# helloybz/CLANE

Measured on AMD Instinct MI355X. Metric: embedding-update iters/sec (Jacobi sweeps of Z <- X + gamma*P*Z, P frozen), higher is better.
Workload: dtype f32; 1 GPU; R-MAT |V|=2000000 |E|=40000000 d=256 f32, gamma=0.76, CosineSimilarity (reference mode), seeds 3/4

## Files before the change

clane_amd/_hip.py:

```python
from __future__ import annotations

import abc
import ctypes as C
import os
import threading
from pathlib import Path
from typing import Optional

import torch

LIB_NAME = "libclane_hip.so"
LIB_PATH = Path(__file__).resolve().parent / LIB_NAME
ABI_VERSION = 5

SCORE_REFERENCE, SCORE_PER_EDGE, SCORE_RAW_DOT = 0, 1, 2
SPMM_SINKS_UNTOUCHED = 1
SPMM_TABLE_BEYOND_CACHE = 2
SCORE_FUSE_SOFTMAX = 1
SCORE_MODES = {"reference": SCORE_REFERENCE, "per_edge": SCORE_PER_EDGE, "raw_dot": SCORE_RAW_DOT}

_p, _i64, _i32 = C.c_void_p, C.c_int64, C.c_int32

SIGNATURES = {
    "clane_abi_version": (C.c_int, []),
    "clane_last_error": (C.c_char_p, []),
    "clane_build_info": (C.c_char_p, []),
    "clane_xcc_ids": (C.c_int, [_p, _i64, _i32, _p]),
    "clane_check_csr": (C.c_int, [_p, _p, _i64, _i64, _i64, _p, _p]),
    "clane_spmm_partials_len": (_i64, [_i64, _i64]),
    "clane_reduce_ws_len": (_i64, []),
    "clane_reduce_partials": (C.c_int, [_p, _i64, _p, _p, _p]),
    "clane_spmm_split_slab_len": (_i64, [_i64, _i32]),
    "clane_spmm_class_slab_len": (_i64, [_i64, _i32]),
    "clane_device_alloc": (C.c_int, [_i64, C.POINTER(_p)]),
    "clane_device_alloc_contiguous": (C.c_int, [_i64, C.POINTER(_p)]),
    "clane_device_free": (C.c_int, [_p]),
    "clane_ipc_export": (C.c_int, [_p, _p]),
    "clane_ipc_open": (C.c_int, [_p, C.POINTER(_p)]),
    "clane_ipc_close": (C.c_int, [_p]),
}
IPC_HANDLE_BYTES = 64
for _s in ("f32", "f64", "bf16"):
    SIGNATURES[f"clane_row_sqnorm_{_s}"] = (C.c_int, [_p, _i64, _i32, _i64, _p, _p])
    SIGNATURES[f"clane_edge_score_{_s}"] = (
        C.c_int, [_p, _p, _i64, _i64, _p, _i64, _i32, _i32, _p, _p, _p, _i32, _i64, _p, _i64, _p])
    _g = C.c_double if _s == "f64" else C.c_float
    SIGNATURES[f"clane_spmm_update_{_s}"] = (
        C.c_int, [_p, _p, _p, _i64, _i64, _p, _i64, _p, _i64, _g, _p, _i64, _i32, _i64, _i32, _p, _p, _p])
    SIGNATURES[f"clane_spmm_update_long_{_s}"] = (
        C.c_int, [_p, _p, _p, _p, _i64, _i32, _i64, _p, _i64, _p, _i64, _g, _p, _i64, _i32, _p, _p, _p])
    SIGNATURES[f"clane_spmm_update_split_{_s}"] = (
        C.c_int,
        [_p, _p, _p, _p, _p, _p, _i64, _i64, _i64, _i64, _p, _i64, _p, _i64, _g, _p, _i64, _i32, _p, _p, _p, _p])
    SIGNATURES[f"clane_spmm_update_class_{_s}"] = (
        C.c_int,
        [_p, _p, _p, _p, _p, _i64, _i32, _p, _p, _i64, _i64, _p, _i64, _p, _i64, _g, _p, _i64, _i32, _i32, _p, _p, _p, _p])
    SIGNATURES[f"clane_edge_score_class_{_s}"] = (
        C.c_int, [_p, _p, _p, _p, _p, _p, _i64, _i32, _p, _p, _i64, _i64, _p, _i64, _i32, _i32, _p, _p, _p, _i32, _p, _p])
    SIGNATURES[f"clane_gather_rows_{_s}"] = (C.c_int, [_p, _i64, _p, _i64, _i32, _p, _i64, _p])
    SIGNATURES[f"clane_l1_distance_{_s}"] = (C.c_int, [_p, _i64, _p, _i64, _i64, _i32, _p, _p, _p, _p])
for _s in ("f32", "f64"):
    SIGNATURES[f"clane_degree_weighted_sums_{_s}"] = (C.c_int, [_p, _p, _p, _i64, _p, _p, _p])
    SIGNATURES[f"clane_edge_score_finalize_{_s}"] = (C.c_int, [_p, _p, _i64, _i64, _i32, _p, _p, _p, _p])
    SIGNATURES[f"clane_segment_softmax_{_s}"] = (C.c_int, [_p, _i64, _p, _i64, _i64, _p, _i64, _p])
    SIGNATURES[f"clane_pair_cosine_{_s}"] = (C.c_int, [_p, _i64, _p, _i64, _i64, _i32, _p, _p, _p])
    SIGNATURES[f"clane_edge_score_pair_{_s}"] = (
        C.c_int, [_p, _p, _i64, _i64, _p, _i64, _p, _i64, _i32, _p, _i32, _i64, _p, _i64, _p])
    SIGNATURES[f"clane_edge_score_class_pair_{_s}"] = (
        C.c_int, [_p, _p, _p, _p, _p, _p, _i64, _i32, _p, _p, _i64, _i64, _p, _i64, _p, _i64, _i32, _p, _i32, _p, _p])
for _s in ("f32", "f64", "bf16"):
    SIGNATURES[f"clane_project_rows_{_s}"] = (C.c_int, [_p, _i64, _i32, _i64, _p, _p, _i64, _p])
    SIGNATURES[f"clane_pair_project_{_s}"] = (C.c_int, [_p, _i64, _i32, _i64, _p, _p, _i64, _p, _p, _p, _p])
    SIGNATURES[f"clane_pair_grad_{_s}"] = (C.c_int, [_p, _i64, _i32, _i64, _p, _p, _i64, _p, _p, _p, _p, _p, _p, _p])
for _s in ("f32", "f64"):
    SIGNATURES[f"clane_pair_loss_{_s}"] = (C.c_int, [_p, _p, _i64, _i32, _p, _p, _p, _p, _p, _p, _p])
    SIGNATURES[f"clane_adam_step_{_s}"] = (C.c_int, [_p, _p, _p, _p, _i64, C.c_double, _p, _p, _p])
SIGNATURES["clane_pair_grad_ws_len"] = (_i64, [_i64, _i32])
RANK_MAX_K = 32
for _s in ("f32", "f64", "bf16"):
    SIGNATURES[f"clane_rank_scores_{_s}"] = (
        C.c_int, [_p, _i64, _p, _i64, _i64, _i32, _p, _i64, _i32, _p, _p, _p, _p, _p, _i32, _i32, _i32, _p, _p, _p])
    SIGNATURES[f"clane_pair_score_{_s}"] = (C.c_int, [_p, _i64, _p, _i64, _i64, _i32, _p, _p, _i64, _i32, _p, _p, _p, _p])
    SIGNATURES[f"clane_rank_count_{_s}"] = (
        C.c_int, [_p, _i64, _p, _i64, _i64, _i32, _p, _p, _i64, _i32, _p, _p, _p, _p, _p, _i32, _i32, _p, _p, _p])
for _s in ("f32", "f64"):
    SIGNATURES[f"clane_rank_merge_{_s}"] = (C.c_int, [_p, _p, _i64, _i32, _i32, _p, _p, _p])
SIGNATURES["clane_pair_labels"] = (C.c_int, [_p, _p, _i64, _p, _p, _i64, _p, _p])
PROBE_MAX_CLASSES = 64
PROBE_WRITE_G, PROBE_WRITE_PRED = 1, 2
PROBE_PRED_TOPK = 4
for _s in ("f32", "f64", "bf16"):
    SIGNATURES[f"clane_probe_forward_{_s}"] = (
        C.c_int, [_p, _i64, _i32, _i64, _p, _p, _i64, _p, _i64, _p, _p, _i32, _i32, _i32, _p, _p, _p, _p, _i64, _p])
    SIGNATURES[f"clane_probe_grad_{_s}"] = (C.c_int, [_p, _i64, _i32, _i64, _p, _i64, _p, _i32, _p, _p, _p, _p])
    SIGNATURES[f"clane_probe_forward_ovr_{_s}"] = (
        C.c_int, [_p, _i64, _i32, _i64, _p, _p, _i64, _p, _i64, _p, _p, _p, _i32, _i32, _i32, _i32, _p, _p, _p, _p, _i64, _p])
SIGNATURES["clane_probe_loss_ws_len"] = (_i64, [_i64, _i32])
SIGNATURES["clane_probe_grad_ws_len"] = (_i64, [_i64, _i32, _i32])
for _s in ("f32", "f64", "bf16"):
    SIGNATURES[f"clane_kmeans_assign_{_s}"] = (
        C.c_int, [_p, _i64, _i32, _i64, _p, _i64, _p, _p, _i32, _i32, _p, _i64, _p, _i64, _p])
    SIGNATURES[f"clane_kmeans_update_{_s}"] = (
        C.c_int, [_p, _i64, _i32, _i64, _p, _p, _i64, _i32, _i32, _p, _p, _p, _p, _p])
SIGNATURES["clane_kmeans_update_ws_len"] = (_i64, [_i64, _i32, _i32, _i32])
for _s in ("f32", "f64", "bf16"):
    _g = C.c_double if _s == "f64" else C.c_float
    SIGNATURES[f"clane_embed_rows_{_s}"] = (
        C.c_int, [_p, _p, _i64, _p, _i64, _p, _i64, _i64, _i32, _i32, _p, _p, _p, _i64, _g, _i32, _i32, _i32, _p, _i64,
                  _p, _p, _p, _p])

PCA_ACCUMULATE = 1
for _s in ("f32", "f64", "bf16"):
    SIGNATURES[f"clane_column_sums_{_s}"] = (C.c_int, [_p, _i64, _i32, _i64, _p, _i64, _i32, _p, _p, _p])
    SIGNATURES[f"clane_gram_{_s}"] = (C.c_int, [_p, _i64, _i32, _i64, _p, _i64, _p, _i32, _p, _p, _p])
    SIGNATURES[f"clane_project_affine_{_s}"] = (C.c_int, [_p, _i64, _i32, _i64, _p, _i64, _p, _p, _i32, _p, _i64, _p])
SIGNATURES["clane_column_sums_ws_len"] = (_i64, [_i64, _i32])
SIGNATURES["clane_gram_ws_len"] = (_i64, [_i64, _i32])


def probe_padded_classes(C_: int) -> int:
    if not 2 <= int(C_) <= PROBE_MAX_CLASSES:
        raise ValueError(f"the label probe handles 2..{PROBE_MAX_CLASSES} classes, got {C_}")
    return 1 << (int(C_) - 1).bit_length()


def ovr_padded_classes(C_: int) -> int:
    if not 1 <= int(C_) <= PROBE_MAX_CLASSES:
        raise ValueError(f"the multi-label probe handles 1..{PROBE_MAX_CLASSES} classes, got {C_}")
    return 1 << (int(C_) - 1).bit_length()


_SUFFIX = {torch.float32: "f32", torch.float64: "f64", torch.bfloat16: "bf16"}
_ACC = {torch.float32: torch.float32, torch.float64: torch.float64, torch.bfloat16: torch.float32}
VEC_ELEMS = {torch.float32: 4, torch.float64: 2, torch.bfloat16: 8}


class ClaneHipError(RuntimeError):
    pass


class _MirrorStruct(C.Structure):
    _fields_ = [("row_ptr", _p), ("slot", _p), ("bufs", _p), ("ld", _i64), ("aligned16", _i32)]

# ... 14 lines not shown
        if len({ld for _, ld in mats}) != 1 or len({b.dtype for b in bufs}) != 1:
            raise ValueError("Mirror: the buffers must share dtype and leading dimension")
        if max(b.shape[0] for b in bufs) > (1 << MIRROR_ROW_BITS):
            raise ValueError("Mirror: a buffer has more than 2^28 rows")
        self.row_ptr, self.slot, self.bufs = row_ptr, slot, bufs
        self.buf = bufs[0]
        self.bases = torch.tensor([ptr for ptr, _ in mats], dtype=torch.int64, device=row_ptr.device)
        self.c = _MirrorStruct(row_ptr.data_ptr(), slot.data_ptr(), self.bases.data_ptr(), mats[0][1],
                               int(all(ptr % 16 == 0 for ptr, _ in mats)))


class _RawDeviceMemory:

    def __init__(self, ptr: int, nbytes: int):
        self.__cuda_array_interface__ = {"shape": (nbytes,), "typestr": "|u1", "data": (ptr, False), "version": 2}


class PeerMatrix:

    def __init__(self, ptr: int, shape, dtype: torch.dtype):
        self._ptr, self.shape, self.dtype = ptr, tuple(shape), dtype

    def data_ptr(self) -> int:
        return self._ptr

    def dim(self) -> int:
        return len(self.shape)

    def stride(self, i: Optional[int] = None):
        st = (self.shape[1], 1)
        return st if i is None else st[i]


class DeviceBuffer:

    def __init__(self, lib, shape, dtype: torch.dtype, device, _mapped_from: Optional[bytes] = None,
                 contiguous: bool = False):
        self.lib, self.shape, self.dtype = lib, tuple(int(x) for x in shape), dtype
        self.nbytes = max(16, int(torch.empty(0, dtype=dtype).element_size()) * int(torch.Size(self.shape).numel()))
        self.mapped = _mapped_from is not None
        ptr = _p()
        with torch.cuda.device(device):
            if self.mapped:
                rc = lib.clane_ipc_open(_mapped_from, C.byref(ptr))
            elif contiguous:
                rc = lib.clane_device_alloc_contiguous(self.nbytes, C.byref(ptr))
            else:
                rc = lib.clane_device_alloc(self.nbytes, C.byref(ptr))
        if rc != 0:
            raise ClaneHipError(f"{'clane_ipc_open' if self.mapped else 'clane_device_alloc'} failed ({rc}): "
                                f"{lib.clane_last_error().decode()}")
        self.ptr = ptr.value
        if self.mapped:
            self.tensor = PeerMatrix(self.ptr, self.shape, dtype)
        else:
            raw = torch.as_tensor(_RawDeviceMemory(self.ptr, self.nbytes), device=torch.device(device))
            n = int(torch.Size(self.shape).numel()) * torch.empty(0, dtype=dtype).element_size()
            self.tensor = raw[:n].view(dtype).view(self.shape)
            self.tensor.zero_()

    def export(self) -> bytes:
        handle = C.create_string_buffer(IPC_HANDLE_BYTES)
        rc = self.lib.clane_ipc_export(self.ptr, handle)
        if rc != 0:
            raise ClaneHipError(f"clane_ipc_export failed ({rc}): {self.lib.clane_last_error().decode()}")
        return handle.raw

    @classmethod
    def open(cls, lib, handle: bytes, shape, dtype: torch.dtype, device) -> "DeviceBuffer":
        return cls(lib, shape, dtype, device, _mapped_from=handle)

    def close(self) -> None:
        if self.ptr:
            (self.lib.clane_ipc_close if self.mapped else self.lib.clane_device_free)(self.ptr)
            self.ptr = 0

    def __del__(self):
        try:
            self.close()
        except Exception:
            pass


def _mirror_arg(mirror: Optional["Mirror"], dtype: torch.dtype):
    if mirror is None:
        return None
    if mirror.buf.dtype != dtype:
        raise ValueError("mirror.buf must have the dtype of Z_new")
    return C.cast(C.pointer(mirror.c), _p)


def load_library(path: Optional[Path] = None) -> C.CDLL:
    if path is None and os.environ.get("CLANE_HIP_LIB"):
        path = os.environ["CLANE_HIP_LIB"]
    path = Path(path) if path is not None else LIB_PATH
    if not path.exists():
        raise ClaneHipError(
            f"{path} not found: the HIP extension is not built. Run `python -c 'import __graft_entry__ as g; "
            f"g.build()'` (or `make -C clane_amd/csrc`) -- clane_amd has no CPU fallback.")
    lib = C.CDLL(str(path))
    for name, (res, args) in SIGNATURES.items():
        fn = getattr(lib, name)
        fn.restype, fn.argtypes = res, args
    got = lib.clane_abi_version()
    if got != ABI_VERSION:
        raise ClaneHipError(f"{path}: ABI version {got}, expected {ABI_VERSION}")
    return lib


def acc_dtype(dtype: torch.dtype) -> torch.dtype:
    try:
        return _ACC[dtype]
    except KeyError:
        raise TypeError(f"clane_amd supports float32, float64 and bfloat16 embeddings, not {dtype}") from None


def _ptr(t: Optional[torch.Tensor]):
    return None if t is None else t.data_ptr()


def _mat(t: torch.Tensor, name: str):
    if t.dim() != 2 or t.stride(1) != 1:
        raise ValueError(f"{name}: need a row-major 2-D tensor with unit column stride, got {tuple(t.shape)} "
                         f"strides {t.stride()}")
    return t.data_ptr(), t.stride(0)


def _vec(t: torch.Tensor, dtype: torch.dtype, name: str):
    if t.dtype != dtype or not t.is_contiguous():
        raise ValueError(f"{name}: need a contiguous {dtype} tensor, got {t.dtype} contiguous={t.is_contiguous()}")
    return t.data_ptr()


class KernelBackend(abc.ABC):

    @abc.abstractmethod
    def spmm_partials_len(self, nrows: int, n_long: int) -> int: ...
    @abc.abstractmethod
    def reduce_ws_len(self) -> int: ...
    @abc.abstractmethod
    def spmm_split_slab_len(self, n_segments: int, d: int) -> int: ...
    @abc.abstractmethod
    def spmm_class_slab_len(self, n_slots: int, d: int) -> int: ...
    @abc.abstractmethod
    def check_csr(self, rowptr, colidx, nrows: int, n_edges: int, table_rows: int) -> None: ...
    @abc.abstractmethod
    def build_info(self) -> str: ...
    @abc.abstractmethod
    def row_sqnorm(self, Z, d: int, sq): ...
    @abc.abstractmethod
    def degree_weighted_sums(self, sq, rowptr, indeg, nrows: int, ws, out2): ...
    @abc.abstractmethod
    def edge_score(self, rowptr, colidx, nrows, row0, Z, d, mode, sums2, sq, scores, long_threshold=0, long_rows=None,
                   fuse_softmax=False): ...
    @abc.abstractmethod
    def edge_score_class(self, rowptr, colidx, item_e0, item_len, item_slot, item_row, items_per_block, class_rows,
                         slot_ptr, row0, Z, d, mode, sums2, sq, scores, stats=None, fuse_softmax=False,
                         n_slots=None, row_parts=1): ...
    @abc.abstractmethod
    def edge_score_finalize(self, rowptr, colidx, nrows, row0, mode, sums2, sq, scores): ...
    @abc.abstractmethod
    def segment_softmax(self, rowptr, nrows, vals, min_degree=0, max_degree=0, long_rows=None): ...
    @abc.abstractmethod
    def pair_cosine(self, A, B, d, out, ws): ...
    @abc.abstractmethod
    def spmm_update(self, rowptr, colidx, P, nrows, row0, Z_old, X, gamma, Z_new, d, long_threshold, partials,
# ... 25 lines not shown
    def project_rows(self, Z, d: int, W, Y):
        raise NotImplementedError(f"{type(self).__name__} has no project_rows")

    def edge_score_pair(self, rowptr, colidx, nrows, row0, S, N, d, scores, long_threshold=0, long_rows=None,
                        fuse_softmax=False):
        raise NotImplementedError(f"{type(self).__name__} has no edge_score_pair")

    def edge_score_class_pair(self, rowptr, colidx, item_e0, item_len, item_slot, item_row, items_per_block,
                              class_rows, slot_ptr, row0, S, N, d, scores, stats=None, fuse_softmax=False,
                              n_slots=None, row_parts=1):
        raise NotImplementedError(f"{type(self).__name__} has no edge_score_class_pair")

    def pair_project(self, Z, d: int, src, dst, W, A, Bm):
        raise NotImplementedError(f"{type(self).__name__} has no pair_project")

    def pair_loss(self, A, Bm, d: int, linked, u, g, mask, ws, stats):
        raise NotImplementedError(f"{type(self).__name__} has no pair_loss")

    def pair_grad_ws_len(self, B: int, d: int) -> int:
        raise NotImplementedError(f"{type(self).__name__} has no pair_grad_ws_len")

    def pair_grad(self, Z, d: int, src, dst, A, Bm, g, stats, ws, dW):
        raise NotImplementedError(f"{type(self).__name__} has no pair_grad")

    def adam_step(self, W, m, v, dW, lr: float, stats, state):
        raise NotImplementedError(f"{type(self).__name__} has no adam_step")

    def pair_labels(self, rowptr, colidx, nrows: int, src, dst, linked):
        raise NotImplementedError(f"{type(self).__name__} has no pair_labels")

    def rank_scores(self, S, N, table_rows: int, d: int, q_rows, mode: int, sums2, sq, label, excl_rowptr, excl_colidx,
                    exclude_self: bool, k: int, n_slabs: int, cand_score, cand_id):
        raise NotImplementedError(f"{type(self).__name__} has no rank_scores")

    def rank_merge(self, cand_score, cand_id, n_slabs: int, k: int, out_score, out_id):
        raise NotImplementedError(f"{type(self).__name__} has no rank_merge")

    def pair_score(self, S, N, table_rows: int, d: int, src, dst, mode: int, sums2, sq, out):
        raise NotImplementedError(f"{type(self).__name__} has no pair_score")

    def rank_count(self, S, N, table_rows: int, d: int, q_rows, t_rows, mode: int, sums2, sq, label, excl_rowptr,
                   excl_colidx, exclude_self: bool, n_slabs: int, target_score, counts):
        raise NotImplementedError(f"{type(self).__name__} has no rank_count")

    def probe_loss_ws_len(self, n: int, F: int) -> int:
        raise NotImplementedError(f"{type(self).__name__} has no probe_loss_ws_len")

    def probe_forward(self, Z, d: int, rows, y, split, W, bias, F: int, C: int, loss_ws, loss, G=None, pred=None):
        raise NotImplementedError(f"{type(self).__name__} has no probe_forward")

    def probe_forward_ovr(self, Z, d: int, rows, ymask, split, W, bias, col_state, F: int, C: int, max_labels: int,
                          loss_ws, loss, G=None, pred=None, top_k: bool = True):
        raise NotImplementedError(f"{type(self).__name__} has no probe_forward_ovr")

    def probe_grad_ws_len(self, n: int, K: int, d: int) -> int:
        raise NotImplementedError(f"{type(self).__name__} has no probe_grad_ws_len")

    def probe_grad(self, Z, d: int, rows, G, ws, dW, db):
        raise NotImplementedError(f"{type(self).__name__} has no probe_grad")

    def kmeans_assign(self, Z, d: int, rows, centres, csq, assign, best):
        raise NotImplementedError(f"{type(self).__name__} has no kmeans_assign")

    def kmeans_update_ws_len(self, n: int, R: int, K: int, d: int) -> int:
        raise NotImplementedError(f"{type(self).__name__} has no kmeans_update_ws_len")

    def kmeans_update(self, Z, d: int, order, seg, centres_old, ws, centres_new, csq_new):
        raise NotImplementedError(f"{type(self).__name__} has no kmeans_update")

    def column_sums_ws_len(self, n: int, d: int) -> int:
        raise NotImplementedError(f"{type(self).__name__} has no column_sums_ws_len")

    def column_sums(self, Z, d: int, rows, ws, sums, accumulate: bool = False):
        raise NotImplementedError(f"{type(self).__name__} has no column_sums")

    def gram_ws_len(self, n: int, d: int) -> int:
        raise NotImplementedError(f"{type(self).__name__} has no gram_ws_len")

    def gram(self, Z, d: int, rows, mu, ws, G, accumulate: bool = False):
        raise NotImplementedError(f"{type(self).__name__} has no gram")

    def project_affine(self, Z, d: int, rows, mu, W, Y):
        raise NotImplementedError(f"{type(self).__name__} has no project_affine")

    def bind(self, method: str, *args, **kwargs):
        fn = getattr(self, method)
        return lambda: fn(*args, **kwargs)

    def embed_rows(self, rowptr, colidx, X_new, Z, table_rows: int, d: int, mode: int, sums2, sq, S, gamma: float,
                   tolerence: int, max_rounds: int, Z_out, rounds, delta, P_out=None, flags: int = 0):
        raise NotImplementedError(f"{type(self).__name__} has no embed_rows")


class HipKernels(KernelBackend):

    def __init__(self, lib: Optional[C.CDLL] = None):
        self.lib = lib if lib is not None else load_library()
        self._tls = threading.local()

    def _invoke(self, fn, what: str, *cargs):
        rec = getattr(self._tls, "recording", None)
        if rec is not None:
            rec.append((fn, cargs, what))
        else:
            self._check(fn(*cargs), what)

    def bind(self, method: str, *args, **kwargs):
        self._tls.recording = []
        try:
            getattr(self, method)(*args, **kwargs)
            (fn, cargs, what), = self._tls.recording
        finally:
            self._tls.recording = None
        check = self._check
        return lambda: check(fn(*cargs), what)

    def _check(self, rc: int, what: str):
        if rc != 0:
            raise ClaneHipError(f"{what} failed ({rc}): {self.lib.clane_last_error().decode()}")

    @staticmethod
    def _stream(t: torch.Tensor):
        if not t.is_cuda:
            raise ClaneHipError("HipKernels needs tensors in GPU memory (got a CPU tensor); there is no CPU path")
        return torch.cuda.current_stream(t.device).cuda_stream

    def _fn(self, base: str, dtype: torch.dtype):
        try:
            return getattr(self.lib, f"{base}_{_SUFFIX[dtype]}")
        except KeyError:
            raise TypeError(f"{base}: unsupported dtype {dtype}") from None

    def spmm_partials_len(self, nrows: int, n_long: int) -> int:
        return int(self.lib.clane_spmm_partials_len(nrows, n_long))

    def xcc_ids(self, n_blocks: int, block_threads: int = 256, device=None) -> torch.Tensor:
        out = torch.full((n_blocks,), -1, dtype=torch.int32, device=device if device is not None else "cuda")
        self._check(self.lib.clane_xcc_ids(out.data_ptr(), n_blocks, block_threads, self._stream(out)), "clane_xcc_ids")
        return out

    def check_csr(self, rowptr: torch.Tensor, colidx: torch.Tensor, nrows: int, n_edges: int, table_rows: int) -> None:
        if rowptr.dtype != torch.int64 or colidx.dtype != torch.int32 or rowptr.numel() < nrows + 1 or colidx.numel() < n_edges:
            raise ValueError("check_csr: rowptr must be int64 [nrows + 1], colidx int32 [n_edges]")
        status = torch.zeros(1, dtype=torch.int32, device=rowptr.device)
        self._check(self.lib.clane_check_csr(rowptr.data_ptr(), colidx.data_ptr(), nrows, n_edges, table_rows,
                                             status.data_ptr(), self._stream(rowptr)), "clane_check_csr")
        bad = int(status.item())
        if bad:
            what = [w for bit, w in ((1, "rowptr is not a non-decreasing sequence within [0, n_edges]"),
                                     (2, f"colidx holds entries outside [0, {table_rows})")) if bad & bit]
            raise ValueError("the CSR handed to the kernels is not valid: " + "; ".join(what))

    def build_info(self) -> str:
        return self.lib.clane_build_info().decode()

    def make_mirror(self, row_ptr, slot, bufs) -> Mirror:
        return Mirror(row_ptr, slot, bufs)

    def reduce_ws_len(self) -> int:
        return int(self.lib.clane_reduce_ws_len())

    def contiguous_matrix(self, shape, dtype: torch.dtype, device) -> DeviceBuffer:
        return DeviceBuffer(self.lib, shape, dtype, device, contiguous=True)

    def shareable_matrix(self, shape, dtype: torch.dtype, device) -> DeviceBuffer:
        return DeviceBuffer(self.lib, shape, dtype, device)
# ... 42 lines not shown
            _vec(scores, acc, "scores"),
            (SCORE_FUSE_SOFTMAX | ((max(1, min(255, int(row_parts))) & 0xff) << 8)) if fuse_softmax else 0,
            None if stats is None else _vec(stats, acc, "stats"), self._stream(Z)), "clane_edge_score_class")

    def edge_score_finalize(self, rowptr, colidx, nrows: int, row0: int, mode: int, sums2, sq, scores):
        self._check(self._fn("clane_edge_score_finalize", scores.dtype)(
            _vec(rowptr, torch.int64, "rowptr"), _vec(colidx, torch.int32, "colidx"), nrows, row0, mode,
            _ptr(sums2), _ptr(sq), scores.data_ptr(), self._stream(scores)), "clane_edge_score_finalize")

    def segment_softmax(self, rowptr, nrows: int, vals, min_degree: int = 0, max_degree: int = 0, long_rows=None):
        n_long = 0 if long_rows is None else long_rows.numel()
        self._check(self._fn("clane_segment_softmax", vals.dtype)(
            _vec(rowptr, torch.int64, "rowptr"), nrows, vals.data_ptr(), min_degree, max_degree,
            None if n_long == 0 else _vec(long_rows, torch.int32, "long_rows"), n_long, self._stream(vals)),
            "clane_segment_softmax")

    @staticmethod
    def _sq_arg(sq: Optional[torch.Tensor], dtype: torch.dtype):
        return None if sq is None else _vec(sq, acc_dtype(dtype), "sq_a")

    def spmm_update(self, rowptr, colidx, P, nrows: int, row0: int, Z_old, X, gamma: float, Z_new, d: int,
                    long_threshold: int, partials, sinks_untouched: bool = False, mirror: Optional[Mirror] = None,
                    beyond_cache: bool = False):
        zo, ldz = _mat(Z_old, "Z_old")
        xp, ldx = _mat(X, "X")
        zn, ldo = _mat(Z_new, "Z_new")
        if not (Z_old.dtype == X.dtype == Z_new.dtype):
            raise ValueError("spmm_update: Z_old, X, Z_new must share a dtype")
        self._invoke(self._fn("clane_spmm_update", Z_old.dtype), "clane_spmm_update",
                     _vec(rowptr, torch.int64, "rowptr"), _vec(colidx, torch.int32, "colidx"),
                     _vec(P, acc_dtype(Z_old.dtype), "P"), nrows, row0, zo, ldz, xp, ldx, gamma, zn, ldo, d,
                     long_threshold, (SPMM_SINKS_UNTOUCHED if sinks_untouched else 0) | (SPMM_TABLE_BEYOND_CACHE if beyond_cache else 0),
                     _mirror_arg(mirror, Z_new.dtype), _vec(partials, torch.float64, "partials"), self._stream(Z_old))

    def spmm_update_long(self, rowptr, colidx, P, long_rows, waves_per_row: int, row0: int, Z_old, X, gamma: float,
                         Z_new, d: int, partials, mirror: Optional[Mirror] = None):
        zo, ldz = _mat(Z_old, "Z_old")
        xp, ldx = _mat(X, "X")
        zn, ldo = _mat(Z_new, "Z_new")
        if not (Z_old.dtype == X.dtype == Z_new.dtype):
            raise ValueError("spmm_update_long: Z_old, X, Z_new must share a dtype")
        self._invoke(self._fn("clane_spmm_update_long", Z_old.dtype), "clane_spmm_update_long",
                     _vec(rowptr, torch.int64, "rowptr"), _vec(colidx, torch.int32, "colidx"),
                     _vec(P, acc_dtype(Z_old.dtype), "P"), _vec(long_rows, torch.int32, "long_rows"),
                     long_rows.numel(), waves_per_row, row0, zo, ldz, xp, ldx, gamma, zn, ldo, d,
                     _mirror_arg(mirror, Z_new.dtype), _vec(partials, torch.float64, "partials"), self._stream(Z_old))

    def spmm_split_slab_len(self, n_segments: int, d: int) -> int:
        return int(self.lib.clane_spmm_split_slab_len(n_segments, d))

    def spmm_update_split(self, rowptr, colidx, P, split_rows, seg_ptr, seg_row, edges_per_segment: int, row0: int,
                          Z_old, X, gamma: float, Z_new, d: int, slab, partials, mirror: Optional[Mirror] = None):
        zo, ldz = _mat(Z_old, "Z_old")
        xp, ldx = _mat(X, "X")
        zn, ldo = _mat(Z_new, "Z_new")
        self._invoke(self._fn("clane_spmm_update_split", Z_old.dtype), "clane_spmm_update_split",
                     _vec(rowptr, torch.int64, "rowptr"), _vec(colidx, torch.int32, "colidx"),
                     _vec(P, acc_dtype(Z_old.dtype), "P"), _vec(split_rows, torch.int32, "split_rows"),
                     _vec(seg_ptr, torch.int64, "seg_ptr"), _vec(seg_row, torch.int32, "seg_row"),
                     split_rows.numel(), seg_row.numel(), edges_per_segment, row0, zo, ldz, xp, ldx, gamma, zn, ldo, d,
                     _vec(slab, acc_dtype(Z_old.dtype), "slab"), _mirror_arg(mirror, Z_new.dtype),
                     _vec(partials, torch.float64, "partials"), self._stream(Z_old))

    def spmm_class_slab_len(self, n_slots: int, d: int) -> int:
        return int(self.lib.clane_spmm_class_slab_len(n_slots, d))

    def spmm_update_class(self, colidx, P, item_e0, item_len, item_slot, items_per_block: int, class_rows, slot_ptr,
                          row0: int, Z_old, X, gamma: float, Z_new, d: int, slab, partials,
                          mirror: Optional[Mirror] = None, beyond_cache: bool = False):
        zo, ldz = _mat(Z_old, "Z_old")
        xp, ldx = _mat(X, "X")
        zn, ldo = _mat(Z_new, "Z_new")
        n_items = item_e0.numel()
        if n_items % items_per_block or item_len.numel() != n_items or item_slot.numel() != n_items:
            raise ValueError("spmm_update_class: the item arrays must hold whole blocks of items_per_block items")
        self._invoke(self._fn("clane_spmm_update_class", Z_old.dtype), "clane_spmm_update_class",
                     _vec(colidx, torch.int32, "colidx"), _vec(P, acc_dtype(Z_old.dtype), "P"),
                     _vec(item_e0, torch.int64, "item_e0"), _vec(item_len, torch.int32, "item_len"),
                     _vec(item_slot, torch.int32, "item_slot"), n_items // items_per_block, items_per_block,
                     _vec(class_rows, torch.int32, "class_rows"), _vec(slot_ptr, torch.int64, "slot_ptr"),
                     class_rows.numel(), row0, zo, ldz, xp, ldx, gamma, zn, ldo, d,
                     SPMM_TABLE_BEYOND_CACHE if beyond_cache else 0,
                     _vec(slab, acc_dtype(Z_old.dtype), "slab"), _mirror_arg(mirror, Z_new.dtype),
                     _vec(partials, torch.float64, "partials"), self._stream(Z_old))

    def reduce_partials(self, partials, n: int, ws, out):
        self._invoke(self.lib.clane_reduce_partials, "clane_reduce_partials",
                     _vec(partials, torch.float64, "partials"), n, _vec(ws, torch.float64, "ws"),
                     _vec(out, torch.float64, "out"), self._stream(out))

    def l1_distance(self, A, B, d: int, ws, out, sq_a: Optional[torch.Tensor] = None):
        ap, lda = _mat(A, "A")
        bp, ldb = _mat(B, "B")
        self._check(self._fn("clane_l1_distance", A.dtype)(
            ap, lda, bp, ldb, A.shape[0], d, self._sq_arg(sq_a, A.dtype), _vec(ws, torch.float64, "ws"),
            _vec(out, torch.float64, "out"), self._stream(A)), "clane_l1_distance")

    def gather_rows(self, src, idx, d: int, dst):
        sp, lds = _mat(src, "src")
        dp, ldd = _mat(dst, "dst")
        self._invoke(self._fn("clane_gather_rows", src.dtype), "clane_gather_rows",
                     sp, lds, _vec(idx, torch.int32, "idx"), idx.numel(), d, dp, ldd, self._stream(src))

    def project_rows(self, Z, d: int, W, Y):
        zp, ldz = _mat(Z, "Z")
        yp, ldy = _mat(Y, "Y")
        acc = acc_dtype(Z.dtype)
        if tuple(W.shape) != (2 * d, d):
            raise ValueError(f"project_rows: W must be [2d, d] = [{2 * d}, {d}], got {tuple(W.shape)}")
        if Y.dtype != acc or Y.shape[0] < Z.shape[0]:
            raise ValueError(f"project_rows: Y must be {acc} with at least {Z.shape[0]} rows")
        self._check(self._fn("clane_project_rows", Z.dtype)(
            zp, Z.shape[0], d, ldz, _vec(W, acc, "W"), yp, ldy, self._stream(Z)), "clane_project_rows")

    def edge_score_pair(self, rowptr, colidx, nrows: int, row0: int, S, N, d: int, scores, long_threshold: int = 0,
                        long_rows=None, fuse_softmax: bool = False):
        sp, lds = _mat(S, "S")
        np_, ldn = _mat(N, "N")
        if S.dtype != N.dtype:
            raise ValueError("edge_score_pair: S and N must share a dtype")
        n_long = 0 if long_rows is None else long_rows.numel()
        self._check(self._fn("clane_edge_score_pair", S.dtype)(
            _vec(rowptr, torch.int64, "rowptr"), _vec(colidx, torch.int32, "colidx"), nrows, row0, sp, lds, np_, ldn, d,
            _vec(scores, S.dtype, "scores"), SCORE_FUSE_SOFTMAX if fuse_softmax else 0, long_threshold,
            None if n_long == 0 else _vec(long_rows, torch.int32, "long_rows"), n_long,
            self._stream(S)), "clane_edge_score_pair")

    def edge_score_class_pair(self, rowptr, colidx, item_e0, item_len, item_slot, item_row, items_per_block: int,
                              class_rows, slot_ptr, row0: int, S, N, d: int, scores, stats=None,
                              fuse_softmax: bool = False, n_slots: Optional[int] = None, row_parts: int = 1):
        sp, lds = _mat(S, "S")
        np_, ldn = _mat(N, "N")
        if S.dtype != N.dtype:
            raise ValueError("edge_score_class_pair: S and N must share a dtype")
        n_items = item_e0.numel()
        if n_items % items_per_block or any(t.numel() != n_items for t in (item_len, item_slot, item_row)):
            raise ValueError("edge_score_class_pair: the item arrays must hold whole blocks of items_per_block items")
        if fuse_softmax and (stats is None or stats.numel() < 2 * (int(slot_ptr[-1]) if n_slots is None else n_slots)):
            raise ValueError("edge_score_class_pair: stats needs 2 elements per slot")
        self._check(self._fn("clane_edge_score_class_pair", S.dtype)(
            _vec(rowptr, torch.int64, "rowptr"), _vec(colidx, torch.int32, "colidx"),
            _vec(item_e0, torch.int64, "item_e0"), _vec(item_len, torch.int32, "item_len"),
            _vec(item_slot, torch.int32, "item_slot"), _vec(item_row, torch.int32, "item_row"),
            n_items // items_per_block, items_per_block, _vec(class_rows, torch.int32, "class_rows"),
            _vec(slot_ptr, torch.int64, "slot_ptr"), class_rows.numel(), row0, sp, lds, np_, ldn, d,
            _vec(scores, S.dtype, "scores"),
            (SCORE_FUSE_SOFTMAX | ((max(1, min(255, int(row_parts))) & 0xff) << 8)) if fuse_softmax else 0,
            None if stats is None else _vec(stats, S.dtype, "stats"), self._stream(S)), "clane_edge_score_class_pair")

    @staticmethod
    def _pairs(src, dst, what: str) -> int:
        if src.numel() != dst.numel():
            raise ValueError(f"{what}: src and dst must have one entry per pair")
        return src.numel()

    def _pair_mats(self, A, Bm, B: int, d: int, acc, what: str):
        for t, name in ((A, "A"), (Bm, "Bm")):
            if t.dtype != acc or not t.is_contiguous() or t.numel() < B * d:
                raise ValueError(f"{what}: {name} must be a contiguous {acc} tensor of at least B * d elements")
        return A.data_ptr(), Bm.data_ptr()

    def pair_project(self, Z, d: int, src, dst, W, A, Bm):
        zp, ldz = _mat(Z, "Z")
        acc = acc_dtype(Z.dtype)
        B = self._pairs(src, dst, "pair_project")
        if tuple(W.shape) != (2 * d, d):
# ... 322 lines not shown
```

clane_amd/csrc/clane_abi.hip:

```cpp
#include "../../include/clane_hip.h"

#include <hip/hip_runtime.h>

#include <climits>
#include <cstdarg>
#include <cstdio>
#include <cstring>

#include "build_p.h"
#include "content_pca.h"
#include "edge_score.h"
#include "device_utils.h"
#include "kmeans.h"
#include "label_probe.h"
#include "multilabel_probe.h"
#include "new_rows.h"
#include "link_eval.h"
#include "link_rank.h"
#include "pair_train.h"
#include "projection.h"
#include "spmm_update.h"

namespace {

// ... 393 lines not shown
        else
            spmm_long_kernel<T, PT, VEC, LPR, U, kLongWaves>
                <<<int(n_long), kLongWaves * kWave, 0, (hipStream_t)stream>>>(
                    rowptr, colidx, P, long_rows, row0, Z_old, ldz, X, ldx, gamma, Z_new, ldo, d, mir, delta_partials);
    });
    return check_launch("spmm_update_long");
}

template <typename T, typename PT>
int spmm_update_split(const int64_t *rowptr, const int32_t *colidx, const PT *P, const int32_t *split_rows,
                      const int64_t *seg_ptr, const int32_t *seg_row, int64_t n_split, int64_t n_segments,
                      int64_t edges_per_segment, int64_t row0, const T *Z_old, int64_t ldz, const T *X, int64_t ldx,
                      typename Elem<T>::acc_t gamma, T *Z_new, int64_t ldo, int32_t d,
                      typename Elem<T>::acc_t *slab, const clane_mirror_t *mirror, double *delta_partials,
                      void *stream) {
    REQUIRE(mirror_ok(mirror, d), "spmm_update_split: incomplete mirror descriptor");
    REQUIRE(n_split >= 0 && n_split <= INT32_MAX && n_segments >= n_split && n_segments <= INT32_MAX && row0 >= 0 &&
                d > 0 && edges_per_segment >= kWave && edges_per_segment % kWave == 0,
            "spmm_update_split: bad shape (edges_per_segment must be a positive multiple of 64)");
    REQUIRE(ldz >= d && ldx >= d && ldo >= d, "spmm_update_split: leading dimension < d");
    if (n_split == 0) return CLANE_OK;
    REQUIRE(rowptr && colidx && P && split_rows && seg_ptr && seg_row && Z_old && X && Z_new && slab && delta_partials,
            "spmm_update_split: null pointer");
    REQUIRE((const void *)Z_new != (const void *)Z_old, "spmm_update_split: Z_new must not alias Z_old");
    REQUIRE(aligned16(slab), "spmm_update_split: slab must be 16-byte aligned");
    const Layout L = pick_layout<T>(d, {Z_old, X, Z_new, mirror_alignment_probe(mirror, Z_new)},
                                    {ldz, ldx, ldo, mirror && mirror->row_ptr ? mirror->ld : ldo});
    const int64_t ld_slab = ceil_div(d, 8) * 8;
    const Mirror<T> mir = make_mirror<T>(mirror);
    dispatch_layout<T>(L, [&]<int VEC, int LPR>() {
        constexpr int U = VEC > 1 ? CLANE_LONG_U : 4;
        spmm_split_segment_kernel<T, PT, VEC, LPR, U, kLongWaves>
            <<<unsigned(n_segments), kLongWaves * kWave, 0, (hipStream_t)stream>>>(
                rowptr, colidx, P, split_rows, seg_ptr, seg_row, edges_per_segment, Z_old, ldz, d, slab, ld_slab);
        spmm_class_combine_kernel<T, VEC, LPR>
            <<<unsigned(ceil_div(n_split, kWave / LPR)), kCombineWaves * kWave, 0, (hipStream_t)stream>>>(
            split_rows, seg_ptr, n_split, row0, slab, ld_slab, Z_old, ldz, X, ldx, gamma, Z_new, ldo, d, mir, false, delta_partials);
    });
    return check_launch("spmm_update_split");
}

template <typename T, typename PT>
int spmm_update_class(const int32_t *colidx, const PT *P, const int64_t *item_e0, const int32_t *item_len,
                      const int32_t *item_slot, int64_t n_blocks, int32_t items_per_block, const int32_t *class_rows,
                      const int64_t *slot_ptr, int64_t n_rows, int64_t row0, const T *Z_old, int64_t ldz, const T *X,
                      int64_t ldx, typename Elem<T>::acc_t gamma, T *Z_new, int64_t ldo, int32_t d, int32_t flags,
                      typename Elem<T>::acc_t *slab, const clane_mirror_t *mirror, double *delta_partials,
                      void *stream) {
    REQUIRE(mirror_ok(mirror, d), "spmm_update_class: incomplete mirror descriptor");
    REQUIRE(n_blocks >= 0 && n_blocks <= INT32_MAX && n_rows >= 0 && n_rows <= INT32_MAX && row0 >= 0 && d > 0,
            "spmm_update_class: bad shape");
    REQUIRE(items_per_block >= kWavesPerBlock && items_per_block <= kMaxItemsPerBlock,
            "spmm_update_class: items_per_block must be in [%d, %d]", kWavesPerBlock, kMaxItemsPerBlock);
    REQUIRE(ldz >= d && ldx >= d && ldo >= d, "spmm_update_class: leading dimension < d");
    if (n_rows == 0) return CLANE_OK;
    REQUIRE(colidx && P && item_e0 && item_len && item_slot && class_rows && slot_ptr && Z_old && X && Z_new && slab &&
                delta_partials,
            "spmm_update_class: null pointer");
    REQUIRE((const void *)Z_new != (const void *)Z_old, "spmm_update_class: Z_new must not alias Z_old");
    REQUIRE(aligned16(slab), "spmm_update_class: slab must be 16-byte aligned");
    const Layout L = pick_layout<T>(d, {Z_old, X, Z_new, mirror_alignment_probe(mirror, Z_new)},
                                    {ldz, ldx, ldo, mirror && mirror->row_ptr ? mirror->ld : ldo});
    const int64_t ld_slab = ceil_div(d, 8) * 8;
    const Mirror<T> mir = make_mirror<T>(mirror);
    dispatch_layout<T>(L, [&]<int VEC, int LPR>() {
        constexpr int U = VEC > 1 ? CLANE_LONG_U : 4;
        constexpr int kDeepU = (LPR == 32 && VEC == 4 && sizeof(T) == 4) ? CLANE_CLASS_U32
                               : (LPR == 16 && VEC == 8 && sizeof(T) == 2) ? CLANE_CLASS_U16B : 0;
        if (n_blocks > 0 && kDeepU > 0 && (flags & CLANE_SPMM_TABLE_BEYOND_CACHE))
            spmm_class_chunk_kernel<T, PT, VEC, LPR, (kDeepU > 0 ? kDeepU : U)>
                <<<unsigned(n_blocks), kBlock, 0, (hipStream_t)stream>>>(
                    colidx, P, item_e0, item_len, item_slot, items_per_block, Z_old, ldz, d, slab, ld_slab);
        else if (n_blocks > 0)
            spmm_class_chunk_kernel<T, PT, VEC, LPR, U><<<unsigned(n_blocks), kBlock, 0, (hipStream_t)stream>>>(
                colidx, P, item_e0, item_len, item_slot, items_per_block, Z_old, ldz, d, slab, ld_slab);
        spmm_class_combine_kernel<T, VEC, LPR>
            <<<unsigned(ceil_div(n_rows, kWave / LPR)), kCombineWaves * kWave, 0, (hipStream_t)stream>>>(
            class_rows, slot_ptr, n_rows, row0, slab, ld_slab, Z_old, ldz, X, ldx, gamma, Z_new, ldo, d, mir,
            (flags & CLANE_SPMM_TABLE_BEYOND_CACHE) != 0, delta_partials);
    });
    return check_launch("spmm_update_class");
}

template <typename T>
int l1_distance(const T *A, int64_t lda, const T *B, int64_t ldb, int64_t nrows, int32_t d,
                typename Elem<T>::acc_t *sq_a, double *ws, double *out, void *stream) {
    REQUIRE(nrows >= 0 && d > 0 && lda >= d && ldb >= d, "l1_distance: bad shape");
    REQUIRE(ws && out, "l1_distance: null workspace/output");
    REQUIRE(nrows == 0 || (A && B), "l1_distance: null pointer");
    const Layout L = pick_layout<T>(d, {A, B}, {lda, ldb});
    if (sq_a != nullptr) {
        const Layout LA = pick_layout<T>(d, {A}, {lda});
        REQUIRE(LA.vec == L.vec && LA.lpr == L.lpr,
                "l1_distance: sq_a needs B as aligned as A (the lane layout of row_sqnorm on A)");
    }
    int grid = 1;
    dispatch_layout<T>(L, [&]<int VEC, int LPR>() {
        grid = grid_for_waves(ceil_div(nrows > 0 ? nrows : 1, (kWave / LPR) * stream_rows(LPR)));
        if (grid > kReduceGrid) grid = kReduceGrid;
        l1_distance_kernel<T, VEC, LPR><<<grid, kBlock, 0, (hipStream_t)stream>>>(A, lda, B, ldb, nrows, d, sq_a, ws);
    });
    reduce_fixed_kernel<<<1, 1024, 0, (hipStream_t)stream>>>(ws, grid, grid, 1, out);
    return check_launch("l1_distance");
}

template <typename T>
int gather_rows(const T *src, int64_t lds, const int32_t *idx, int64_t n, int32_t d, T *dst, int64_t ldd, void *stream) {
    REQUIRE(n >= 0 && d > 0 && lds >= d && ldd >= d, "gather_rows: bad shape");
    if (n == 0) return CLANE_OK;
    REQUIRE(src && idx && dst, "gather_rows: null pointer");
    const Layout L = pick_layout<T>(d, {src, dst}, {lds, ldd});
    dispatch_layout<T>(L, [&]<int VEC, int LPR>() {
        const int grid = grid_for_waves(ceil_div(n, kWave / LPR));
        gather_rows_kernel<T, VEC, LPR><<<grid, kBlock, 0, (hipStream_t)stream>>>(src, lds, idx, n, d, dst, ldd);
    });
    return check_launch("gather_rows");
}

template <typename T>
int pair_cosine(const T *A, int64_t lda, const T *B, int64_t ldb, int64_t nrows, int32_t d,
                typename Elem<T>::acc_t *out, double *ws, void *stream) {
    REQUIRE(nrows >= 0 && d > 0 && lda >= d && ldb >= d, "pair_cosine: bad shape");
    if (nrows == 0) return CLANE_OK;
    REQUIRE(A && B && out && ws, "pair_cosine: null pointer");
    const Layout L = pick_layout<T>(d, {A, B}, {lda, ldb});
    int grid = 1;
    dispatch_layout<T>(L, [&]<int VEC, int LPR>() {
        grid = grid_for_waves(ceil_div(nrows, kWave / LPR));
        if (grid > kReduceGrid) grid = kReduceGrid;
        pair_dot_kernel<T, VEC, LPR><<<grid, kBlock, 0, (hipStream_t)stream>>>(A, lda, B, ldb, nrows, d, out, ws);
    });
    double *sums2 = ws + 2 * kReduceGrid;
    reduce_fixed_kernel<<<1, 1024, 0, (hipStream_t)stream>>>(ws, grid, grid, 2, sums2);
    int sgrid = int(ceil_div(nrows, kBlock));
    if (sgrid > kMaxGrid) sgrid = kMaxGrid;
    pair_scale_kernel<typename Elem<T>::acc_t><<<sgrid, kBlock, 0, (hipStream_t)stream>>>(out, nrows, sums2);
    return check_launch("pair_cosine");
}

template <typename T, typename A>
int pair_project(const T *Z, int64_t table_rows, int32_t d, int64_t ldz, const int32_t *src, const int32_t *dst,
                 int64_t B, const A *W, A *PA, A *PB, void *stream) {
    REQUIRE(table_rows >= 0 && B >= 0 && d > 0 && d <= 32768 && ldz >= d, "pair_project: bad shape rows=%lld B=%lld d=%d ldz=%lld",
            (long long)table_rows, (long long)B, d, (long long)ldz);
    if (B == 0) return CLANE_OK;
    REQUIRE(Z && src && dst && W && PA && PB, "pair_project: null pointer");
    const int n_tiles = int(ceil_div(int64_t(d), int64_t(kProjBN)));
    const int64_t blocks = ceil_div(B, int64_t(kProjBM)) * n_tiles;
    REQUIRE(blocks <= INT32_MAX, "pair_project: %lld pairs is too many for one launch", (long long)B);
    pair_project_kernel<T, A><<<dim3(unsigned(blocks), 2), kBlock, 0, (hipStream_t)stream>>>(
        Z, table_rows, d, ldz, src, dst, B, W, PA, PB, n_tiles);
    return check_launch("pair_project");
}

template <typename A>
int pair_loss(const A *PA, const A *PB, int64_t B, int32_t d, const uint8_t *linked, const A *u, A *g, uint8_t *mask,
              double *ws, double *stats, void *stream) {
    REQUIRE(B >= 0 && d > 0, "pair_loss: bad shape B=%lld d=%d", (long long)B, d);
    REQUIRE(ws && stats, "pair_loss: null workspace/output");
    REQUIRE(B == 0 || (PA && PB && linked && u && g && mask), "pair_loss: null pointer");
    int grid = int(ceil_div(B > 0 ? B : 1, kBlock / kPairLanes));
    if (grid > kReduceGrid) grid = kReduceGrid;
    pair_loss_kernel<A><<<grid, kBlock, 0, (hipStream_t)stream>>>(PA, PB, B, d, linked, u, g, mask, ws);
    reduce_fixed_kernel<<<1, 1024, 0, (hipStream_t)stream>>>(ws, grid, grid, 2, stats);
    return check_launch("pair_loss");
}
// ... 547 lines not shown
        return edge_score_pair<T>(rowptr, colidx, nrows, row0, S, lds, N, ldn, d, scores, flags, long_threshold,      \
                                  long_rows, n_long, stream);                                                          \
    }                                                                                                                  \
    int clane_edge_score_class_pair_##SUF(const int64_t *rowptr, const int32_t *colidx, const int64_t *item_e0,        \
                                          const int32_t *item_len, const int32_t *item_slot, const int32_t *item_row,  \
                                          int64_t n_blocks, int32_t items_per_block, const int32_t *class_rows,        \
                                          const int64_t *slot_ptr, int64_t n_rows, int64_t row0, const T *S,           \
                                          int64_t lds, const T *N, int64_t ldn, int32_t d, T *scores, int32_t flags,   \
                                          T *stats, void *stream) {                                                    \
        return edge_score_class_pair<T>(rowptr, colidx, item_e0, item_len, item_slot, item_row, n_blocks,             \
                                        items_per_block, class_rows, slot_ptr, n_rows, row0, S, lds, N, ldn, d,       \
                                        scores, flags, stats, stream);                                                 \
    }
CLANE_EDGE_SCORE_PAIR_WRAPPERS(f32, float)
CLANE_EDGE_SCORE_PAIR_WRAPPERS(f64, double)
#undef CLANE_EDGE_SCORE_PAIR_WRAPPERS

int clane_edge_score_finalize_f32(const int64_t *rowptr, const int32_t *colidx, int64_t nrows, int64_t row0,
                                  int32_t mode, const double *sums2, const float *sq, float *scores, void *stream) {
    return edge_score_finalize<float>(rowptr, colidx, nrows, row0, mode, sums2, sq, scores, stream);
}
int clane_edge_score_finalize_f64(const int64_t *rowptr, const int32_t *colidx, int64_t nrows, int64_t row0,
                                  int32_t mode, const double *sums2, const double *sq, double *scores, void *stream) {
    return edge_score_finalize<double>(rowptr, colidx, nrows, row0, mode, sums2, sq, scores, stream);
}
int clane_segment_softmax_f32(const int64_t *rowptr, int64_t nrows, float *vals, int64_t min_degree,
                              int64_t max_degree, const int32_t *long_rows, int64_t n_long, void *stream) {
    return segment_softmax<float>(rowptr, nrows, vals, min_degree, max_degree, long_rows, n_long, stream);
}
int clane_segment_softmax_f64(const int64_t *rowptr, int64_t nrows, double *vals, int64_t min_degree,
                              int64_t max_degree, const int32_t *long_rows, int64_t n_long, void *stream) {
    return segment_softmax<double>(rowptr, nrows, vals, min_degree, max_degree, long_rows, n_long, stream);
}

#define CLANE_SPMM_WRAPPERS(SUF, CT, T, PT, GT)                                                                        \
    int clane_spmm_update_##SUF(const int64_t *rowptr, const int32_t *colidx, const PT *P, int64_t nrows,             \
                                int64_t row0, const CT *Z_old, int64_t ldz, const CT *X, int64_t ldx, GT gamma,       \
                                CT *Z_new, int64_t ldo, int32_t d, int64_t long_threshold, int32_t flags,             \
                                const clane_mirror_t *mirror, double *delta_partials, void *stream) {                \
        return spmm_update<T, PT>(rowptr, colidx, P, nrows, row0, reinterpret_cast<const T *>(Z_old), ldz,            \
                                  reinterpret_cast<const T *>(X), ldx, gamma, reinterpret_cast<T *>(Z_new), ldo, d,   \
                                  long_threshold, flags, mirror, delta_partials, stream);                             \
    }                                                                                                                 \
    int clane_spmm_update_long_##SUF(const int64_t *rowptr, const int32_t *colidx, const PT *P,                       \
                                     const int32_t *long_rows, int64_t n_long, int32_t waves_per_row, int64_t row0, const CT *Z_old,         \
                                     int64_t ldz, const CT *X, int64_t ldx, GT gamma, CT *Z_new, int64_t ldo,         \
                                     int32_t d, const clane_mirror_t *mirror, double *delta_partials, void *stream) { \
        return spmm_update_long<T, PT>(rowptr, colidx, P, long_rows, n_long, waves_per_row, row0,                     \
                                       reinterpret_cast<const T *>(Z_old), ldz, reinterpret_cast<const T *>(X), ldx,  \
                                       gamma, reinterpret_cast<T *>(Z_new), ldo, d, mirror, delta_partials, stream);  \
    }
#define CLANE_SPLIT_WRAPPER(SUF, CT, T, PT, GT)                                                                         \
    int clane_spmm_update_split_##SUF(const int64_t *rowptr, const int32_t *colidx, const PT *P,                      \
                                      const int32_t *split_rows, const int64_t *seg_ptr, const int32_t *seg_row,      \
                                      int64_t n_split, int64_t n_segments, int64_t edges_per_segment, int64_t row0,   \
                                      const CT *Z_old, int64_t ldz, const CT *X, int64_t ldx, GT gamma, CT *Z_new,    \
                                      int64_t ldo, int32_t d, GT *slab, const clane_mirror_t *mirror,                 \
                                      double *delta_partials, void *stream) {                                         \
        return spmm_update_split<T, PT>(rowptr, colidx, P, split_rows, seg_ptr, seg_row, n_split, n_segments,         \
                                        edges_per_segment, row0, reinterpret_cast<const T *>(Z_old), ldz,             \
                                        reinterpret_cast<const T *>(X), ldx, gamma, reinterpret_cast<T *>(Z_new),     \
                                        ldo, d, slab, mirror, delta_partials, stream);                                \
    }
CLANE_SPLIT_WRAPPER(f32, float, float, float, float)
CLANE_SPLIT_WRAPPER(f64, double, double, double, double)
CLANE_SPLIT_WRAPPER(bf16, uint16_t, bf16_t, float, float)
#undef CLANE_SPLIT_WRAPPER
#define CLANE_CLASS_WRAPPER(SUF, CT, T, PT, GT)                                                                        \
    int clane_spmm_update_class_##SUF(const int32_t *colidx, const PT *P, const int64_t *item_e0,                     \
                                      const int32_t *item_len, const int32_t *item_slot, int64_t n_blocks,            \
                                      int32_t items_per_block, const int32_t *class_rows, const int64_t *slot_ptr,    \
                                      int64_t n_rows, int64_t row0, const CT *Z_old, int64_t ldz, const CT *X,        \
                                      int64_t ldx, GT gamma, CT *Z_new, int64_t ldo, int32_t d, int32_t flags,        \
                                      GT *slab, const clane_mirror_t *mirror, double *delta_partials, void *stream) { \
        return spmm_update_class<T, PT>(colidx, P, item_e0, item_len, item_slot, n_blocks, items_per_block,           \
                                        class_rows, slot_ptr, n_rows, row0, reinterpret_cast<const T *>(Z_old), ldz,  \
                                        reinterpret_cast<const T *>(X), ldx, gamma, reinterpret_cast<T *>(Z_new),     \
                                        ldo, d, flags, slab, mirror, delta_partials, stream);                         \
    }
CLANE_CLASS_WRAPPER(f32, float, float, float, float)
CLANE_CLASS_WRAPPER(f64, double, double, double, double)
CLANE_CLASS_WRAPPER(bf16, uint16_t, bf16_t, float, float)
#undef CLANE_CLASS_WRAPPER
int64_t clane_spmm_class_slab_len(int64_t n_slots, int32_t d) { return n_slots * (ceil_div(d, 8) * 8); }
int64_t clane_spmm_split_slab_len(int64_t n_segments, int32_t d) { return n_segments * (ceil_div(d, 8) * 8); }

CLANE_SPMM_WRAPPERS(f32, float, float, float, float)
CLANE_SPMM_WRAPPERS(f64, double, double, double, double)
CLANE_SPMM_WRAPPERS(bf16, uint16_t, bf16_t, float, float)
#undef CLANE_SPMM_WRAPPERS

int clane_reduce_partials(const double *partials, int64_t n, double *ws, double *out, void *stream) {
    if (n < 0 || !out || !ws || (n > 0 && !partials))
        return fail(CLANE_ERR_INVALID_ARGUMENT, "reduce_partials: bad arguments");
    if (n <= 8192) {
        reduce_fixed_kernel<<<1, 1024, 0, (hipStream_t)stream>>>(partials, n, n, 1, out);
    } else {
        const int64_t slice = ceil_div(n, kReduceGrid);
        const int grid = int(ceil_div(n, slice));
        reduce_slices_kernel<<<grid, kBlock, 0, (hipStream_t)stream>>>(partials, n, slice, ws);
        reduce_fixed_kernel<<<1, 1024, 0, (hipStream_t)stream>>>(ws, grid, grid, 1, out);
    }
    return check_launch("reduce_partials");
}

int clane_l1_distance_f32(const float *A, int64_t lda, const float *B, int64_t ldb, int64_t nrows, int32_t d,
                          float *sq_a, double *ws, double *out, void *stream) {
    return l1_distance<float>(A, lda, B, ldb, nrows, d, sq_a, ws, out, stream);
}
int clane_l1_distance_f64(const double *A, int64_t lda, const double *B, int64_t ldb, int64_t nrows, int32_t d,
                          double *sq_a, double *ws, double *out, void *stream) {
    return l1_distance<double>(A, lda, B, ldb, nrows, d, sq_a, ws, out, stream);
}
int clane_l1_distance_bf16(const uint16_t *A, int64_t lda, const uint16_t *B, int64_t ldb, int64_t nrows, int32_t d,
                           float *sq_a, double *ws, double *out, void *stream) {
    return l1_distance<bf16_t>(reinterpret_cast<const bf16_t *>(A), lda, reinterpret_cast<const bf16_t *>(B), ldb,
                               nrows, d, sq_a, ws, out, stream);
}

int clane_gather_rows_f32(const float *src, int64_t lds, const int32_t *idx, int64_t n, int32_t d, float *dst,
                          int64_t ldd, void *stream) {
    return gather_rows<float>(src, lds, idx, n, d, dst, ldd, stream);
}
int clane_gather_rows_f64(const double *src, int64_t lds, const int32_t *idx, int64_t n, int32_t d, double *dst,
                          int64_t ldd, void *stream) {
    return gather_rows<double>(src, lds, idx, n, d, dst, ldd, stream);
}
int clane_gather_rows_bf16(const uint16_t *src, int64_t lds, const int32_t *idx, int64_t n, int32_t d, uint16_t *dst,
                           int64_t ldd, void *stream) {
    return gather_rows<bf16_t>(reinterpret_cast<const bf16_t *>(src), lds, idx, n, d,
                               reinterpret_cast<bf16_t *>(dst), ldd, stream);
}

int clane_pair_cosine_f32(const float *A, int64_t lda, const float *B, int64_t ldb, int64_t nrows, int32_t d,
                          float *out, double *ws, void *stream) {
    return pair_cosine<float>(A, lda, B, ldb, nrows, d, out, ws, stream);
}
int clane_pair_cosine_f64(const double *A, int64_t lda, const double *B, int64_t ldb, int64_t nrows, int32_t d,
                          double *out, double *ws, void *stream) {
    return pair_cosine<double>(A, lda, B, ldb, nrows, d, out, ws, stream);
}

#define CLANE_PAIR_TRAIN_WRAPPERS(SUF, CT, T, AT)                                                                      \
    int clane_pair_project_##SUF(const CT *Z, int64_t table_rows, int32_t d, int64_t ldz, const int32_t *src,         \
                                 const int32_t *dst, int64_t B, const AT *W, AT *A, AT *Bm, void *stream) {           \
        return pair_project<T, AT>(reinterpret_cast<const T *>(Z), table_rows, d, ldz, src, dst, B, W, A, Bm,         \
                                   stream);                                                                           \
    }                                                                                                                 \
    int clane_pair_grad_##SUF(const CT *Z, int64_t table_rows, int32_t d, int64_t ldz, const int32_t *src,            \
                              const int32_t *dst, int64_t B, const AT *A, const AT *Bm, const AT *g,                  \
                              const double *stats, AT *ws, AT *dW, void *stream) {                                    \
        return pair_grad<T, AT>(reinterpret_cast<const T *>(Z), table_rows, d, ldz, src, dst, B, A, Bm, g, stats, ws, \
                                dW, stream);                                                                          \
    }
CLANE_PAIR_TRAIN_WRAPPERS(f32, float, float, float)
CLANE_PAIR_TRAIN_WRAPPERS(f64, double, double, double)
CLANE_PAIR_TRAIN_WRAPPERS(bf16, uint16_t, bf16_t, float)
#undef CLANE_PAIR_TRAIN_WRAPPERS
#define CLANE_PAIR_LOSS_WRAPPERS(SUF, AT)                                                                              \
    int clane_pair_loss_##SUF(const AT *A, const AT *Bm, int64_t B, int32_t d, const uint8_t *linked, const AT *u,    \
                              AT *g, uint8_t *mask, double *ws, double *stats, void *stream) {                        \
        return pair_loss<AT>(A, Bm, B, d, linked, u, g, mask, ws, stats, stream);                                     \
    }                                                                                                                 \
    int clane_adam_step_##SUF(AT *W, AT *m, AT *v, const AT *dW, int64_t n, double lr, const double *stats,           \
                              double *state, void *stream) {                                                          \
        return adam_step<AT>(W, m, v, dW, n, lr, stats, state, stream);                                               \
// ... 148 lines not shown
```

clane_amd/csrc/spmm_update.h:

```cpp
#pragma once

#include "device_utils.h"

#ifndef CLANE_SPMM_U
#define CLANE_SPMM_U 8
#endif
#ifndef CLANE_SPMM_DYNAMIC
#define CLANE_SPMM_DYNAMIC 1
#endif
#ifndef CLANE_COMBINE_WAVES
#define CLANE_COMBINE_WAVES 2
#endif
#ifndef CLANE_SPMM_PREFETCH
#define CLANE_SPMM_PREFETCH 1
#endif
#ifndef CLANE_SPMM_MIN_WAVES
#define CLANE_SPMM_MIN_WAVES 0
#endif

namespace clane {

template <typename A>
struct EdgeChunk {
    int c;
// ... 646 lines not shown

constexpr int kCombineWaves = CLANE_COMBINE_WAVES;
#ifndef CLANE_COMBINE_LOADS
#define CLANE_COMBINE_LOADS 16
#endif
constexpr int kCombineLoads = CLANE_COMBINE_LOADS;

template <typename T, int VEC, int LPR>
__global__ __launch_bounds__(kCombineWaves *kWave) void spmm_class_combine_kernel(
    const int32_t *__restrict__ class_rows, const int64_t *__restrict__ slot_ptr, int64_t n_rows, int64_t row0,
    const typename Elem<T>::acc_t *__restrict__ slab, int64_t ld_slab, const T *__restrict__ Zold, int64_t ldz,
    const T *__restrict__ X, int64_t ldx, typename Elem<T>::acc_t gamma, T *__restrict__ Znew, int64_t ldo, int d,
    Mirror<T> mirror, bool nt_store, double *__restrict__ partials) {
    using A = typename Elem<T>::acc_t;
    constexpr int kRows = kWave / LPR;
    __shared__ A s_part[kCombineWaves > 1 ? kCombineWaves - 1 : 1][kWave][VEC];
    const int lane = lane_id();
    const int wave = __builtin_amdgcn_readfirstlane(threadIdx.x / kWave);
    const int sub = lane / LPR, sl = lane % LPR;
    const int64_t i = int64_t(blockIdx.x) * kRows + sub;
    const bool live = i < n_rows;
    const int64_t r = live ? class_rows[i] : 0;
    const int64_t s0 = live ? slot_ptr[i] : 0, s1 = live ? slot_ptr[i + 1] : 0;
    const int64_t share = ceil_div(s1 - s0, int64_t(kCombineWaves));
    const int64_t a = s0 + wave * share < s1 ? s0 + wave * share : s1;
    const int64_t b = a + share < s1 ? a + share : s1;
    A rsum = A(0);
    for (int t0 = 0; t0 < d; t0 += LPR * VEC) {
        const int c0 = t0 + sl * VEC;
        const bool ok = live && c0 < d;
        A acc[VEC];
#pragma unroll
        for (int k = 0; k < VEC; ++k) acc[k] = A(0);
        if (ok) {
            int64_t s = a;
            for (; s + kCombineLoads <= b; s += kCombineLoads) {
                Pack<A, VEC> part[kCombineLoads];
#pragma unroll
                for (int u = 0; u < kCombineLoads; ++u) part[u] = slab_load<A, VEC>(slab + (s + u) * ld_slab + c0);
#pragma unroll
                for (int u = 0; u < kCombineLoads; ++u) {
#pragma unroll
                    for (int k = 0; k < VEC; ++k) acc[k] += part[u].v[k];
                }
            }
#pragma unroll 4
            for (; s < b; ++s) {
                const Pack<A, VEC> part = slab_load<A, VEC>(slab + s * ld_slab + c0);
#pragma unroll
                for (int k = 0; k < VEC; ++k) acc[k] += part.v[k];
            }
        }
        if constexpr (kCombineWaves > 1) {
            if (t0 > 0) __syncthreads();
            if (wave > 0) {
#pragma unroll
                for (int k = 0; k < VEC; ++k) s_part[wave - 1][lane][k] = acc[k];
            }
            __syncthreads();
        }
        if (wave == 0) {
            Pack<T, VEC> out{};
            if (ok) {
                if constexpr (kCombineWaves > 1) {
#pragma unroll
                    for (int w = 1; w < kCombineWaves; ++w) {
#pragma unroll
                        for (int k = 0; k < VEC; ++k) acc[k] += s_part[w - 1][lane][k];
                    }
                }
                const Pack<T, VEC> x = load_pack_stream<T, VEC>(X + r * ldx + c0);
                const Pack<T, VEC> zo = load_pack_stream<T, VEC>(Zold + (row0 + r) * ldz + c0);
                rsum += finish_pack<T, VEC>(x, zo, acc, gamma, true, Znew + r * ldo + c0, out, nt_store);
            }
            if (live) mirror_store<T, VEC, LPR>(mirror, r, c0, out, ok, sl, sub * LPR);
        }
    }
    if (wave == 0) {
        rsum = group_sum<LPR>(rsum);
        if (live && sl == 0) partials[i] = double(rsum);
    }
}

}
```

clane_amd/diagnostics.py:

```python
from __future__ import annotations

import numpy as np

from .plan import lanes_per_row


class DiagnosticsMixin:

    def kernel_times_ms(self):
        t = np.array([(e0.elapsed_time(e4), e4.elapsed_time(e1), e1.elapsed_time(e2), e2.elapsed_time(e3))
                      for _, e0, e1, e2, e3, e4 in self.kernel_events]).reshape(-1, 4)
        self.kernel_events = []
        if not len(t):
            return {}
        per_sweep = t.reshape(-1, len(self.blocks), 4).sum(1).mean(0)
        return dict(zip(("split", "hub", "mid", "main"), per_sweep.tolist()))

    def collective_times_ms(self):
        ev, self.collective_events = self.collective_events, []
        if not ev:
            return {}
        t = np.array([(a.elapsed_time(b), b.elapsed_time(c)) for a, b, c in ev])
        return {"exchange_exposed": float(t[:, 0].mean()), "allreduce": float(t[:, 1].mean()), "sweeps_timed": len(ev)}

    def kernel_bytes(self):
        s, ps = self.Zcur.element_size(), self.P.element_size()
        deg = np.diff(self.local.rowptr)
        per_row = deg * (self.d * s + 4 + ps) + np.where(deg > 0, 3 * self.d * s, 0) + 8
        is_long = deg > self.long_threshold if self.long_threshold > 0 else np.zeros_like(deg, dtype=bool)
        is_class = deg > self.class_threshold if self.class_threshold > 0 else np.zeros_like(deg, dtype=bool)
        is_long = is_long | is_class
        is_split = (is_long & (deg > self.split_edges) if self.split_edges > 0 else np.zeros_like(is_long)) & ~is_class
        is_hub = is_long & (deg > self.hub_threshold) & ~is_split & ~is_class
        return {"main": int(per_row[~is_long].sum()) + 8,
                "mid": int(per_row[is_long & ~is_hub & ~is_split & ~is_class].sum()),
                "hub": int(per_row[is_hub].sum()), "split": int(per_row[is_split | is_class].sum())}

    def launches_per_sweep(self) -> int:
        return len(self.blocks) * len(self.tiles)

    def kernel_names(self):
        narrow = self.d > 0 and lanes_per_row(self.d_plan if len(self.tiles) > 1 else self.d, self.dtype) < 64
        return {"main": "spmm_update_subrow_kernel" if narrow else "spmm_update_kernel",
                "mid": "spmm_long_kernel<4 waves>", "hub": "spmm_long_kernel<16 waves>",
                "split": "spmm_class_chunk_kernel+combine" if self.class_threshold > 0
                else "spmm_split_segment_kernel+combine"}

    def estimated_sweep_seconds(self) -> float:
        s = self.Zcur.element_size()
        d = self.d_full
        total = self.E_total * (d * s + 8) + self.V * 3 * d * s
        return total / max(self.world, 1) / 8e12

    def kernel_config(self) -> dict:
        return {"build": self.k.build_info(), "dtype": str(self.dtype).replace("torch.", ""), "d": self.d,
                "lanes_per_row": lanes_per_row(self.d, self.dtype) if self.d > 0 else 0,
                "rows": int(self.part.n_local), "edges": int(self.E_loc), "launch_blocks": len(self.blocks),
                "long_threshold": self.long_threshold, "score_threshold": self.score_threshold,
                "hub_threshold": self.hub_threshold,
                "split_edges": self.split_edges, "segment_edges": self.segment_edges,
                "class_threshold": self.class_threshold, "class_chunk": self.class_chunk, "class_k1": self.class_k1,
                "class_phases": self.class_phases, "phase_threshold": self.phase_threshold,
                "class_of_row": "xor-fold of 3-bit groups" if self.class_threshold else None,
                "class_affinity": self.class_affinity, "mega_segment_edges": self.mega_segment_edges,
                "class_items_per_block": [c[6] for c in self.class_rows if c is not None][:1],
                "column_tiles": len(self.tiles),
                "fewer_loads_in_flight": bool(self.beyond_cache and self.d > 0 and (str(self.dtype), lanes_per_row(
                    self.d_plan if len(self.tiles) > 1 else self.d, self.dtype)) in (("torch.float32", 32), ("torch.bfloat16", 16))),
                "hot_rows_first": self.hot_rows_first, "exchange": self.exchange,
                }

    def exchange_bytes_per_sweep(self) -> int:
        s = self.Zcur.element_size()
        if self.halo:
            return self.part.recv_rows_per_sweep() * self.ld * s
        if self.columns:
            return 0
        return sum((b.span[1] - b.span[0] - b.nrows) * self.ld * s for b in self.blocks if b.span is not None)
```

clane_amd/engine.py:

```python
from __future__ import annotations

import contextlib
import threading
from typing import List, Optional

import numpy as np
import torch

from . import _hip, xcd
from .comm import TorchComm
from .diagnostics import DiagnosticsMixin
from .halo import build_halo_layout
from .partition import Block, HostCSR, LocalCSR, RowPartition, localize
from .plan import (HEAVY_ROW_EDGES, HUB_FACTOR, INFINITY_CACHE_BYTES, L2_BYTES_ALL_XCDS,
                   LONG_THRESHOLD_BY_ROWS_PER_WAVE, MIN_HOT_READ_SHARE, MIN_SEGMENT_EDGES, MIN_SLICE_ROW_BYTES,
                   SOFTMAX_EDGES_PER_WORKGROUP, SPLIT_EDGES, TARGET_SEGMENTS, UNSKEWED_LONG_THRESHOLD, _round_up,
                   column_slice, hot_read_share, lanes_per_row, pick_exchange)
from .staging import StagedZ, StagingMixin, place_piece
from .xcd import (CLASS_CHUNK, CLASS_THRESHOLD_BY_ROWS_PER_WAVE, PHASE_THRESHOLD, PHASES_BY_ROWS_PER_WAVE,
                  class_items)

class SweepEngine(StagingMixin, DiagnosticsMixin):
    STAGE_SLOTS = 3
    N_TABLES = 3
    MAX_TIMED_SWEEPS = 32

    EXCHANGES = ("auto", "columns", "halo", "halo_p2p", "allgather", "allgather_all")

    def __init__(self, csr: HostCSR, X: torch.Tensor, device, kernels=None, *, cosine_mode: str = "reference",
                 process_group=None, chunks: Optional[int] = None, long_threshold: Optional[int] = None,
                 hub_threshold: Optional[int] = None, shuffle: Optional[bool] = None, seed: int = 0,
                 exchange: str = "auto", comm=None, hot_rows_first: bool = True, split_hubs: bool = True,
                 overlap_chunks: bool = True, fused_pack: bool = True, class_threshold: Optional[int] = None,
                 class_chunk: int = CLASS_CHUNK, class_k1: bool = True, class_phases: Optional[int] = None,
                 phase_threshold: int = PHASE_THRESHOLD, delta_stream: bool = False, table_skew=None,
                 table_alloc: str = "torch", column_tiles: Optional[int] = None):
        if X.dim() != 2 or X.shape[0] != csr.num_vertices:
            raise ValueError(f"X must be [V, d] with V={csr.num_vertices}, got {tuple(X.shape)}")
        if cosine_mode not in ("reference", "per_edge"):
            raise ValueError(f"cosine_mode must be 'reference' or 'per_edge', got {cosine_mode!r}")
        csr.validate()
        csr.indeg(device)
        self.k = kernels if kernels is not None else _hip.kernels()
        self.device = torch.device(device)
        self.dtype = X.dtype
        self.acc_dtype = _hip.acc_dtype(X.dtype)
        self.cosine_mode = cosine_mode
        self.table_skew = table_skew
        if table_alloc not in ("torch", "contiguous"):
            raise ValueError("table_alloc must be 'torch' or 'contiguous'")
        self.table_alloc, self._own_tables, self.table_alloc_note = table_alloc, [], None
        self._column_tiles_asked = column_tiles
        X = self._choose_division(csr, X, process_group, comm, exchange)
        self._choose_class_pass(csr, class_threshold, class_chunk, class_k1, class_phases, phase_threshold)
        self._build_layout(csr, chunks, shuffle, seed, hot_rows_first)
        self._choose_row_bins(long_threshold, hub_threshold)
        deg = self._upload_structure()
        self._bin_rows(deg, split_hubs)
        self._setup_exchange(deg, fused_pack)
        self._alloc_tables(X, deg)
        self._alloc_scratch(delta_stream, overlap_chunks)
        self._Y = None

    def _choose_division(self, csr: HostCSR, X: torch.Tensor, process_group, comm, exchange: str) -> torch.Tensor:
        self.pg = process_group
        self.comm = comm if comm is not None else (TorchComm(process_group) if process_group is not None else None)
        self.world = self.comm.world if self.comm is not None else 1
        rank = self.comm.rank if self.comm is not None else 0
        if exchange not in self.EXCHANGES:
            raise ValueError("exchange must be 'auto', 'columns', 'halo', 'halo_p2p', 'allgather' or "
                             f"'allgather_all', got {exchange!r}")
        self._forced = self.world == 1 and self.comm is not None and bool(self.comm.force) and exchange in (
            "columns", "allgather", "allgather_all")
        divided = self.world > 1 or self._forced
        if exchange == "auto":
            exchange = pick_exchange(int(X.shape[1]), X.dtype, self.world)
        self._exchange_asked = exchange
        self.exchange = exchange if divided else "none"
        self.columns = divided and exchange == "columns"
        self.C = self.world if self.columns else 1
        self.c = rank if self.columns else 0
        self.V, self.d_full = csr.num_vertices, int(X.shape[1])
        self.E_total = csr.num_edges
        self.col0, self.col1 = column_slice(self.d_full, X.dtype, self.C, self.c) if self.columns else (0, self.d_full)
        if self.columns:
            X = X[:, self.col0:self.col1]
            self.ld_max = _round_up(column_slice(self.d_full, X.dtype, self.C, 0)[1], _hip.VEC_ELEMS[X.dtype])
        self.d = self.col1 - self.col0
        self.ld = _round_up(self.d, _hip.VEC_ELEMS[X.dtype])
        self.row_world, self.row_rank = (1, 0) if self.columns else (self.world, rank)
        self.halo = self.row_world > 1 and exchange in ("halo", "halo_p2p")
        self.p2p = self.halo and exchange == "halo_p2p"
        if self.p2p and self.world > 8:
            raise ValueError("halo_p2p addresses at most 8 GPUs (one box)")
        self.d_plan = self.d
        if self.columns:
            c0, c1 = column_slice(self.d_full, X.dtype, self.C, 0)
            self.d_plan = c1 - c0
        T = self._pick_tiles(csr, X.dtype) if not divided else 1
        cuts = [column_slice(self.d, X.dtype, T, t) for t in range(T)] if self.d > 0 else [(0, 0)]
        self.tiles = [c for c in cuts if c[1] > c[0]] or [(0, self.d)]
        if len(self.tiles) > 1:
            self.d_plan = max(c1 - c0 for c0, c1 in self.tiles)
        self.beyond_cache = csr.num_vertices * self.ld * torch.empty(0, dtype=X.dtype).element_size() > 2 * INFINITY_CACHE_BYTES
        self.ld_plan = _round_up(self.d_plan, _hip.VEC_ELEMS[X.dtype])
        self.rows_per_wave = 64 // lanes_per_row(self.d_plan, X.dtype) if self.d_plan > 0 else 1
        return X

    def _pick_tiles(self, csr: HostCSR, dtype: torch.dtype) -> int:
        asked = self._column_tiles_asked
        if asked is not None:
            if asked < 1:
                raise ValueError("column_tiles must be >= 1")
            return int(asked)
        if dtype != torch.float32 or self.d < 256 or self.d % 128:
            return 1
        if csr.num_vertices * self.ld * 4 <= 2 * INFINITY_CACHE_BYTES:
            return 1
        return min(8, self.d // 128) if hot_read_share(csr, 512) >= MIN_HOT_READ_SHARE else 1

    def _choose_class_pass(self, csr: HostCSR, class_threshold, class_chunk, class_k1, class_phases,
                           phase_threshold) -> None:
        row_bytes = self.ld_plan * torch.empty(0, dtype=self.dtype).element_size()
        self.hot_read_share = hot_read_share(csr, row_bytes) if self.d_plan > 0 else 1.0
        self.class_affinity = True
        if class_threshold is None:
            class_threshold = CLASS_THRESHOLD_BY_ROWS_PER_WAVE[self.rows_per_wave]
            if self.rows_per_wave == 2 and csr.num_vertices * row_bytes <= INFINITY_CACHE_BYTES:
                class_threshold = max(class_threshold, 128)
            if self.hot_read_share < MIN_HOT_READ_SHARE:
                class_threshold = max(class_threshold, HEAVY_ROW_EDGES)
                self.class_affinity = False
        self.class_threshold = int(class_threshold)
        self.class_chunk = int(class_chunk)
        self.class_k1 = bool(class_k1) and self.class_threshold > 0
        if class_phases is None:
            class_phases = (xcd.PHASES_UNDER_COLUMN_TILES if len(self.tiles) > 1 else 0) or \
                PHASES_BY_ROWS_PER_WAVE[self.rows_per_wave]
        self.class_phases = int(class_phases)
        if self.class_threshold == 0 or self.class_phases < 1:
            self.class_phases = 1
        if self.class_phases & (self.class_phases - 1) or self.class_phases > 8:
            raise ValueError("class_phases must be 1, 2, 4 or 8")
        self.phase_threshold = max(int(phase_threshold), self.class_threshold) if self.class_phases > 1 else 0
        if self.class_threshold and not (64 <= self.class_chunk <= 4096 and self.class_chunk % 64 == 0):
            raise ValueError("class_chunk must be a multiple of 64 in [64, 4096]")
        self.mega_segment_edges = int(L2_BYTES_ALL_XCDS // 8 // max(row_bytes, 1)) if self.d_plan > 0 else 0

    def _build_layout(self, csr: HostCSR, chunks, shuffle, seed: int, hot_rows_first: bool) -> None:
        if chunks is None:
            chunks = 1 if self.row_world == 1 else 4
        self.hot_rows_first = bool(hot_rows_first)
        if self.halo:
            self.part = build_halo_layout(csr, self.row_world, self.row_rank, chunks, shuffle=shuffle is not False, seed=seed,
                                          hot_rows_first=hot_rows_first, class_threshold=self.class_threshold,
                                          phase_threshold=self.phase_threshold, phases=self.class_phases)
            self.blocks: List[Block] = self.part.blocks
            self.local: LocalCSR = self.part.local
        else:
            live = csr.live_mask() if (self.row_world > 1 and self._exchange_asked == "allgather") else None
            hot = csr.indeg() if (self.row_world == 1 and hot_rows_first and not shuffle) else None
            self.part = RowPartition.create(self.V, self.row_world, self.row_rank, chunks, live_mask=live, shuffle=shuffle,
                                            seed=seed, priority=hot)
            self.blocks = self.part.blocks(spans_for_one_rank=self._forced and not self.columns)
            self.local = localize(csr, self.part, self.device, class_threshold=self.class_threshold,
                                  phase_threshold=self.phase_threshold, phases=self.class_phases)
        if self.part.padded_vertices >= 2 ** 31:
            raise ValueError(f"{self.part.padded_vertices} table rows: column indices are 32-bit (ABI v1); divide the "
                             "rows over more GPUs (exchange='halo') or wait for 64-bit indices")

    def _choose_row_bins(self, long_threshold, hub_threshold) -> None:
        if long_threshold is None:
            long_threshold = LONG_THRESHOLD_BY_ROWS_PER_WAVE[self.rows_per_wave]
            if self.rows_per_wave == 1 and self.class_threshold and self.class_affinity:
                long_threshold = max(long_threshold, self.class_threshold)
            elif self.rows_per_wave == 1 and not self.class_affinity:
                long_threshold = max(long_threshold, UNSKEWED_LONG_THRESHOLD)
            if self.rows_per_wave > 1:
                by_size = 1 << max(7, int(self.local.colidx.shape[0] // 32768).bit_length() - 1)
                long_threshold = min(long_threshold, by_size)
        self.score_threshold = int(long_threshold)
        self.k1_threshold = (min(self.score_threshold, self.class_threshold) if self.score_threshold > 0
                             else self.class_threshold) if self.class_k1 else self.score_threshold
        if self.class_threshold:
            long_threshold = min(long_threshold, self.class_threshold) if long_threshold > 0 else self.class_threshold
        self.long_threshold = int(long_threshold)
        self.hub_threshold = int(hub_threshold) if hub_threshold is not None else HUB_FACTOR * self.long_threshold

    def _upload_structure(self) -> np.ndarray:
        dev = self.device
        self.rowptr = torch.from_numpy(self.local.rowptr).to(dev)
        self.colidx = torch.from_numpy(self.local.colidx).to(dev)
        if self.colidx.numel() == 0:
            self.colidx = torch.zeros(1, dtype=torch.int32, device=dev)
        self.indeg = torch.from_numpy(self.local.indeg).to(dev)
        self.E_loc = int(self.local.colidx.shape[0])
        self.k.check_csr(self.rowptr, self.colidx, self.part.n_local, self.E_loc, self.part.padded_vertices)
        self.P = torch.zeros(max(self.E_loc, 1), dtype=self.acc_dtype, device=dev)
        self.P_valid = False
        deg = np.diff(self.local.rowptr)
        self.max_degree = int(deg.max()) if deg.size else 0
        self.softmax_row_parts = int(min(64, max(1, -(-self.max_degree // SOFTMAX_EDGES_PER_WORKGROUP))))
        return deg

    def _bin_rows(self, deg: np.ndarray, split_hubs: bool) -> None:
        dev = self.device
        self.long_rows: List[Optional[torch.Tensor]] = []
        self.mid_rows: List[Optional[torch.Tensor]] = []
        self.hub_rows: List[Optional[torch.Tensor]] = []
        self.split_rows: List[Optional[tuple]] = []
        self.class_rows: List[Optional[tuple]] = []
        self.class_slots: List[int] = []
        self.k1_long_rows: List[Optional[torch.Tensor]] = []
        self.split_edges = SPLIT_EDGES if split_hubs else 0
        hub_edges = int(deg[deg > SPLIT_EDGES].sum()) // max(1, len(self.blocks))
        self.segment_edges = int(min(SPLIT_EDGES, max(MIN_SEGMENT_EDGES, hub_edges // TARGET_SEGMENTS // 1024 * 1024)))
        max_segments = max_slots = 0
        self.partial_off = [0]
        to_dev = lambda a: torch.from_numpy(a.astype(np.int32)).to(dev) if a.size else None
        for b in self.blocks:
            db = deg[b.local_start:b.local_start + b.nrows]
            is_long = db > self.long_threshold if self.long_threshold > 0 else np.zeros_like(db, dtype=bool)
            is_class = db > self.class_threshold if self.class_threshold > 0 else np.zeros_like(db, dtype=bool)
            is_long = is_long | is_class
            is_split = (is_long & (db > self.split_edges) if self.split_edges > 0 else np.zeros_like(is_long)) & ~is_class
            is_hub = is_long & (db > self.hub_threshold) & ~is_split & ~is_class
            self.long_rows.append(to_dev(np.nonzero(db > self.score_threshold)[0] if self.score_threshold > 0
                                         else np.empty(0, dtype=np.int64)))
            self.mid_rows.append(to_dev(np.nonzero(is_long & ~is_hub & ~is_split & ~is_class)[0]))
            rows_c = np.nonzero(is_class)[0]
            if rows_c.size:
                rows_abs = rows_c + b.local_start
                phased = dict(phase_threshold=self.phase_threshold, phases=self.class_phases,
                              mega_segment_edges=self.mega_segment_edges,
                              mega_min_edges=self.part.padded_vertices // 4)
                items = class_items(self.local.rowptr, self.local.colidx, rows_abs, self.class_chunk, None,
                                    row_ids=rows_c, colidx_dev=self.colidx, **phased)
                ipb = items["items_per_block"]
                self.class_rows.append((to_dev(rows_c), torch.from_numpy(items["slot_ptr"]).to(dev),
                                        torch.from_numpy(items["e0"]).to(dev), torch.from_numpy(items["len"]).to(dev),
                                        torch.from_numpy(items["slot"]).to(dev), torch.from_numpy(items["row"]).to(dev),
                                        ipb))
                self.class_slots.append(int(items["slot_ptr"][-1]))
                max_slots = max(max_slots, self.class_slots[-1])
            else:
                self.class_rows.append(None)
                self.class_slots.append(0)
            k1_long = (db > self.k1_threshold) & ~(is_class if self.class_k1 else np.zeros_like(is_class)) \
                if self.k1_threshold > 0 else np.zeros_like(is_class)
            self.k1_long_rows.append(to_dev(np.nonzero(k1_long)[0]))
            self.hub_rows.append(to_dev(np.nonzero(is_hub)[0]))
            rows_s = np.nonzero(is_split)[0]
            if rows_s.size:
                nseg = -(-db[rows_s] // self.segment_edges)
                seg_ptr = np.zeros(rows_s.size + 1, dtype=np.int64)
                np.cumsum(nseg, out=seg_ptr[1:])
                seg_row = np.repeat(np.arange(rows_s.size, dtype=np.int32), nseg)
                self.split_rows.append((to_dev(rows_s), torch.from_numpy(seg_ptr).to(dev),
                                        torch.from_numpy(seg_row).to(dev)))
                max_segments = max(max_segments, int(seg_ptr[-1]))
            else:
                self.split_rows.append(None)
            self.partial_off.append(self.partial_off[-1] + self.k.spmm_partials_len(b.nrows, int(is_long.sum())))
        self.partials = torch.zeros(self.partial_off[-1] * len(self.tiles), dtype=torch.float64, device=dev)
        slab_len = max(1, self.k.spmm_split_slab_len(max_segments, max(self.d_plan, 1)))
        if max_slots:
            slab_len = max(slab_len, self.k.spmm_class_slab_len(max_slots, max(self.d_plan, 1)), 2 * max_slots)
        self.slabs = [torch.zeros(slab_len, dtype=self.acc_dtype, device=dev)
                      for _ in range(2 if len(self.blocks) > 1 else 1)]

    def _setup_exchange(self, deg: np.ndarray, fused_pack: bool) -> None:
        dev = self.device
        self.send_rows: List[Optional[torch.Tensor]] = []
        self.send_buf: List[Optional[torch.Tensor]] = []
        self.mirrors: List[Optional[object]] = []
        self.fused_pack = bool(fused_pack)
        for b in self.blocks:
            ex = b.exchange
            has = ex is not None and ex.send_rows.size > 0 and not self.p2p
            self.send_rows.append(torch.from_numpy(ex.send_rows).to(dev) if has else None)
            self.send_buf.append(torch.zeros(ex.send_rows.size, self.ld, dtype=self.dtype, device=dev) if has
                                 else (torch.zeros(0, self.ld, dtype=self.dtype, device=dev) if ex is not None else None))
            mirror = None
            if has and self.fused_pack:
                rel = ex.send_rows.astype(np.int64) - b.local_start
                if rel.min() < 0 or rel.max() >= b.nrows or (deg[ex.send_rows] == 0).any():
                    raise AssertionError("halo send list holds a row outside its chunk or a row that never changes")
                row_ptr = np.zeros(b.nrows + 1, dtype=np.int64)
                np.cumsum(np.bincount(rel, minlength=b.nrows), out=row_ptr[1:])
                slot = np.argsort(rel, kind="stable").astype(np.int32)
                mirror = self._make_mirror(torch.from_numpy(row_ptr).to(dev), torch.from_numpy(slot).to(dev),
                                           self.send_buf[-1])
            self.mirrors.append(mirror)

    def _new_table(self, tag: str, rows: int) -> torch.Tensor:
        skew = (self.table_skew or {}).get(tag)
        if self.table_alloc == "contiguous":
            try:
                buf = self.k.contiguous_matrix((rows, self.ld), self.dtype, self.device)
                self._own_tables.append(buf)
                return buf.tensor
            except _hip.ClaneHipError as exc:
                self.table_alloc_note = f"{tag}: {exc}"
        if skew is None or self.device.type != "cuda":
            return torch.zeros(rows, self.ld, dtype=self.dtype, device=self.device)
        es = torch.empty(0, dtype=self.dtype).element_size()
        nbytes = rows * self.ld * es
        raw = torch.zeros(nbytes + (4 << 20) + int(skew), dtype=torch.uint8, device=self.device)
        start = (-raw.data_ptr()) % (2 << 20) + int(skew)
        return raw[start:start + nbytes].view(self.dtype).view(rows, self.ld)

    def _alloc_tables(self, X: torch.Tensor, deg: np.ndarray) -> None:
        dev = self.device
        if self.halo:
            self.table_vertex = torch.from_numpy(self.part.table_vertex).to(dev)
            self.slot = torch.from_numpy(self.part.vertex_slot).to(dev)
        else:
            self.pos = torch.from_numpy(self.part.position_of_vertex()).to(dev)
        if self.p2p:
            self._shared = [self.k.shareable_matrix((self.part.padded_vertices, self.ld), self.dtype, dev)
                            for _ in range(self.N_TABLES)]
            self.Zbuf = [b.tensor for b in self._shared]
            self.peer_tables, self._mapped = self.comm.share_matrices(self.k, self._shared)
            self._build_p2p_mirrors(deg)
        else:
            self.Zbuf = [self._new_table(f"Z{i}", self.part.padded_vertices) for i in range(2)]
        self.cur, self.hold, self._prev_cur, self._tick = 0, None, 0, 0
        Xd = X.to(dev)
        verts = torch.from_numpy(self.local.vertex).to(dev)
        ok = verts >= 0
        self.X_loc = self._new_table("X", self.part.n_local)
        self.X_loc[ok, :self.d] = Xd[verts[ok]]
        self.quiet_stale = False
        self._load_Z(Xd)

    def _alloc_scratch(self, delta_stream: bool, overlap_chunks: bool) -> None:
        dev = self.device
        self.ws = torch.zeros(self.k.reduce_ws_len(), dtype=torch.float64, device=dev)
        self.sums2 = torch.zeros(2, dtype=torch.float64, device=dev)
        self.delta = torch.zeros(1, dtype=torch.float64, device=dev)
        self.delta_pp = torch.zeros(2, dtype=torch.float64, device=dev)
        self._delta_host = torch.zeros(2, dtype=torch.float64)
        self._delta_ev = None
        if self.device.type == "cuda":
            self._delta_host = self._delta_host.pin_memory()
            self._delta_ev = [torch.cuda.Event() for _ in range(2)]
        self._delta_stream = None
        self._delta_busy = [False, False]
        if self.device.type == "cuda" and (self.world > 1 or self._forced) and delta_stream:
            self._delta_stream = torch.cuda.Stream(self.device)
        self.block_out = torch.zeros(len(self.blocks), dtype=torch.float64, device=dev)
        self.sq_pp = [torch.zeros(self.part.n_local, dtype=self.acc_dtype, device=dev) for _ in self.Zbuf]
# ... 149 lines not shown
                k.row_sqnorm(Z, self.d, self.sq_full)
            if self.columns:
                self._all_reduce(self.sq_full)
            sq = self.sq_full
        if self.E_loc > 0 and not self.columns:
            for i, b in enumerate(self.blocks):
                rp = self.rowptr[b.local_start:]
                k.edge_score(rp, self.colidx, b.nrows, b.row0, Z, self.d, mode, self.sums2, sq, self.P,
                             self.k1_threshold, self.k1_long_rows[i], fuse_softmax=True)
                if self.class_k1 and self.class_rows[i] is not None:
                    rows_c, slot_ptr, it_e0, it_len, it_slot, it_row, ipb = self.class_rows[i]
                    k.edge_score_class(rp, self.colidx, it_e0, it_len, it_slot, it_row, ipb, rows_c,
                                       slot_ptr, b.row0, Z, self.d, mode, self.sums2, sq, self.P,
                                       self.slabs[i % len(self.slabs)], fuse_softmax=True,
                                       n_slots=self.class_slots[i], row_parts=self.softmax_row_parts)
        elif self.E_loc > 0:
            if busy:
                for i, b in enumerate(self.blocks):
                    k.edge_score(self.rowptr[b.local_start:], self.colidx, b.nrows, b.row0, Z, self.d,
                                 _hip.SCORE_RAW_DOT, None, None, self.P, self.k1_threshold, self.k1_long_rows[i])
                    if self.class_k1 and self.class_rows[i] is not None:
                        rows_c, slot_ptr, it_e0, it_len, it_slot, it_row, ipb = self.class_rows[i]
                        k.edge_score_class(self.rowptr[b.local_start:], self.colidx, it_e0, it_len, it_slot, it_row,
                                           ipb, rows_c, slot_ptr, b.row0, Z, self.d,
                                           _hip.SCORE_RAW_DOT, None, None, self.P)
            else:
                self.P.zero_()
            self._all_reduce(self.P)
            for i, b in enumerate(self.blocks):
                rp = self.rowptr[b.local_start:]
                k.edge_score_finalize(rp, self.colidx, b.nrows, b.row0, mode, self.sums2, sq, self.P)
                k.segment_softmax(rp, b.nrows, self.P, 0, self.score_threshold if self.long_rows[i] is not None else 0,
                                  self.long_rows[i])
        self.P_valid = True

    def build_P_bilinear(self, W: torch.Tensor) -> None:
        from .bilinear import build_P_bilinear
        build_P_bilinear(self, W)

    def similarity_trainer(self, W0: torch.Tensor, lr: float, batch_size: int = 4):
        from .train import SimilarityTrainer
        return SimilarityTrainer(self, W0, lr, batch_size)

    def set_cosine_mode(self, mode: str) -> None:
        if mode not in ("reference", "per_edge"):
            raise ValueError(f"cosine_mode must be 'reference' or 'per_edge', got {mode!r}")
        if mode != self.cosine_mode:
            self.cosine_mode, self.P_valid = mode, False

    def P_global(self) -> torch.Tensor:
        out = torch.zeros(int(self.local.edge_origin.max()) + 1 if self.E_loc else 0, dtype=self.acc_dtype)
        out[torch.from_numpy(self.local.edge_origin)] = self.P[:self.E_loc].to("cpu")
        return out

    def _bind(self, method: str, *args, **kwargs):
        return self.k.bind(method, *args, **kwargs)

    def _build_plan(self, cur: int, dst: int, tick: int, gamma: float):
        k = self.k
        Zold, Znew = self.Zbuf[cur], self.Zbuf[dst]
        per_block = []
        for i, b in enumerate(self.blocks):
            steps = []
            ctx = torch.cuda.stream(self.side_streams[i % 2]) if self.side_streams else contextlib.nullcontext()
            with ctx:
                rp, Xb, Zn = self.rowptr[b.local_start:], self.X_loc[self._rows(b)], self._zrows(Znew, b)
                po = self.partial_off[i]
                mir = self.mirrors_p2p[dst][i] if self.p2p else self.mirrors[i]
                po_mid = po + k.spmm_partials_len(b.nrows, 0)
                po_hub = po_mid + (0 if self.mid_rows[i] is None else self.mid_rows[i].numel())
                po_split = po_hub + (0 if self.hub_rows[i] is None else self.hub_rows[i].numel())
                po_class = po_split + (0 if self.split_rows[i] is None else self.split_rows[i][0].numel())
                steps.append(("event", i, 0))
                if self.d == 0:
                    per_block.append(steps + [("event", i, e) for e in (4, 1, 2, 3)])
                    continue
                T = len(self.tiles)
                cut = (lambda M, t: M) if T == 1 else (lambda M, t: M[:, self.tiles[t][0]:self.tiles[t][1]])
                width = (lambda t: self.d) if T == 1 else (lambda t: self.tiles[t][1] - self.tiles[t][0])
                part = lambda off, t: self.partials[t * self.partial_off[-1] + off:]
                if mir is not None and T > 1:
                    raise AssertionError("column tiles and mirrored launches do not combine")
                for t in range(T):
                    if self.class_rows[i] is not None:
                        rows_c, slot_ptr, it_e0, it_len, it_slot, _, ipb = self.class_rows[i]
                        steps.append(("call", self._bind("spmm_update_class", self.colidx, self.P, it_e0, it_len, it_slot,
                                                         ipb, rows_c, slot_ptr, b.row0, cut(Zold, t), cut(Xb, t), gamma,
                                                         cut(Zn, t), width(t), self.slabs[i % len(self.slabs)],
                                                         part(po_class, t), mirror=mir, beyond_cache=self.beyond_cache)))
                    if self.split_rows[i] is not None:
                        rows_s, seg_ptr, seg_row = self.split_rows[i]
                        steps.append(("call", self._bind("spmm_update_split", rp, self.colidx, self.P, rows_s, seg_ptr,
                                                         seg_row, self.segment_edges, b.row0, cut(Zold, t), cut(Xb, t), gamma,
                                                         cut(Zn, t), width(t), self.slabs[i % len(self.slabs)],
                                                         part(po_split, t), mirror=mir)))
                steps.append(("event", i, 4))
                for t in range(T):
                    if self.hub_rows[i] is not None:
                        steps.append(("call", self._bind("spmm_update_long", rp, self.colidx, self.P, self.hub_rows[i], 16,
                                                         b.row0, cut(Zold, t), cut(Xb, t), gamma, cut(Zn, t), width(t),
                                                         part(po_hub, t), mirror=mir)))
                steps.append(("event", i, 1))
                for t in range(T):
                    if self.mid_rows[i] is not None:
                        steps.append(("call", self._bind("spmm_update_long", rp, self.colidx, self.P, self.mid_rows[i], 4,
                                                         b.row0, cut(Zold, t), cut(Xb, t), gamma, cut(Zn, t), width(t),
                                                         part(po_mid, t), mirror=mir)))
                steps.append(("event", i, 2))
                for t in range(T):
                    steps.append(("call", self._bind("spmm_update", rp, self.colidx, self.P, b.nrows, b.row0, cut(Zold, t),
                                                     cut(Xb, t), gamma, cut(Zn, t), width(t), self.long_threshold,
                                                     part(po, t), sinks_untouched=True, mirror=mir,
                                                     beyond_cache=self.beyond_cache)))
                steps.append(("event", i, 3))
                if b.span is not None:
                    steps.append(("allgather", Znew[b.span[0]:b.span[1]], Zn))
                elif b.exchange is not None and not self.p2p:
                    ex = b.exchange
                    if self.send_rows[i] is not None and mir is None:
                        steps.append(("call", self._bind("gather_rows", Znew, self.send_rows[i], self.d,
                                                         self.send_buf[i])))
                    steps.append(("alltoall", Znew[ex.recv_start:ex.recv_start + ex.recv_rows], self.send_buf[i],
                                  ex.out_splits, ex.in_splits))
            per_block.append(steps)
        final = self._bind("reduce_partials", self.partials, self.partials.numel(), self.ws,
                           self.delta_pp[tick:tick + 1])
        return per_block, final

    def sweep(self, gamma: float) -> float:
        return self.sweep_wait(self.sweep_launch(gamma))

    def sweep_launch(self, gamma: float) -> int:
        if not self.P_valid:
            raise RuntimeError("sweep() before build_P()")
        stream = torch.cuda.current_stream(self.device).cuda_stream if self.device.type == "cuda" else 0
        src = self.cur
        dst = next(i for i in range(len(self.Zbuf)) if i != src and i != self.hold)
        parity = self._tick
        self._tick ^= 1
        if self._delta_stream is not None and self._delta_busy[parity]:
            torch.cuda.current_stream(self.device).wait_event(self._delta_ev[parity])
            self._delta_busy[parity] = False
        key = (src, dst, parity, float(gamma), stream)
        plan = self._plans.get(key)
        if plan is None:
            plan = self._plans[key] = self._build_plan(src, dst, parity, float(gamma))
        events = None
        if self.time_kernels and len(self.kernel_events) < self.MAX_TIMED_SWEEPS * len(self.blocks):
            events = [[torch.cuda.Event(enable_timing=True) for _ in range(5)] for _ in self.blocks]
            self.kernel_events.extend((i,) + tuple(ev) for i, ev in enumerate(events))
        per_block, final = plan
        works = []
        side = self.side_streams
        if side:
            main = torch.cuda.current_stream(self.device)
            start = torch.cuda.Event()
            start.record(main)
            for st in side:
                st.wait_event(start)
        for i, steps in enumerate(per_block):
            ctx = torch.cuda.stream(side[i % 2]) if side else contextlib.nullcontext()
            with ctx:
                for step in steps:
                    kind = step[0]
                    if kind == "call":
                        step[1]()
                    elif kind == "event":
# ... 84 lines not shown
```

clane_amd/xcd.py:

```python
from __future__ import annotations

from typing import Optional

import numpy as np
import torch

XCD_CLASSES = 8


def xcd_class(position):
    p = position
    return (p ^ (p >> 3) ^ (p >> 6) ^ (p >> 9)) & (XCD_CLASSES - 1)


def xcd_subclass(position, row_degree, class_threshold: int, phase_threshold: int = 0, phases: int = 1):
    cls = xcd_class(position)
    if phases > 1 and phase_threshold > 0:
        cls = cls + XCD_CLASSES * (((position >> 6) % phases) * (row_degree > phase_threshold))
    return cls * (row_degree > class_threshold)


CLASS_THRESHOLD_BY_ROWS_PER_WAVE = {1: 64, 2: 64, 4: 256, 8: 256}
CLASS_CHUNK = 256
PHASES_BY_ROWS_PER_WAVE = {1: 4, 2: 2, 4: 1, 8: 1}
PHASES_UNDER_COLUMN_TILES = 0
PHASE_THRESHOLD = 512
CLASS_ITEMS_PIECE_EDGES = 1 << 28
CLASS_ITEMS_PER_BLOCK = 16



def row_pieces(rowptr: np.ndarray, max_edges: int):
    n = rowptr.size - 1
    a = 0
    while a < n:
        b = int(np.searchsorted(rowptr, rowptr[a] + max_edges, side="right")) - 1
        b = min(max(b, a + 1), n)
        yield a, b
        a = b


def class_items(rowptr: np.ndarray, colidx: np.ndarray, rows: np.ndarray, chunk: int, items_per_block: Optional[int],
                row_ids: Optional[np.ndarray] = None, colidx_dev: Optional[torch.Tensor] = None,
                phase_threshold: int = 0, phases: int = 1, mega_segment_edges: int = 0, mega_min_edges: int = 0) -> dict:
    n = rows.size
    NS = XCD_CLASSES * max(1, phases)
    sizes = (rowptr[rows + 1] - rowptr[rows]).astype(np.int64)
    start = np.concatenate([[0], np.cumsum(sizes)[:-1]])
    if colidx_dev is not None and colidx_dev.is_cuda:
        dev = colidx_dev.device
        seg_len = np.empty(n * NS, dtype=np.int64)
        unsorted = False
        bounds = np.concatenate([[0], np.cumsum(sizes)])
        for a, b in row_pieces(bounds, CLASS_ITEMS_PIECE_EDGES):
            if bounds[b] == bounds[a]:
                seg_len[a * NS:b * NS] = 0
                continue
            sizes_t = torch.from_numpy(sizes[a:b]).to(dev)
            rid = torch.repeat_interleave(torch.arange(b - a, device=dev), sizes_t)
            idx = (torch.from_numpy(rowptr[rows[a:b]] - (start[a:b] - bounds[a])).to(dev)[rid]
                   + torch.arange(int(bounds[b] - bounds[a]), device=dev))
            sub = xcd_subclass(colidx_dev[idx].long(), sizes_t[rid], 0, phase_threshold, phases)
            key = rid * NS + sub
            unsorted = unsorted or (bool((key[1:] < key[:-1]).any()) if key.numel() > 1 else False)
            seg_len[a * NS:b * NS] = torch.bincount(key, minlength=(b - a) * NS).cpu().numpy()
    else:
        idx = np.repeat(rowptr[rows] - start, sizes) + np.arange(int(sizes.sum()), dtype=np.int64)
        rid = np.repeat(np.arange(n, dtype=np.int64), sizes)
        sub = xcd_subclass(colidx[idx].astype(np.int64), sizes[rid], 0, phase_threshold, phases)
        unsorted = idx.size > 1 and bool((np.diff(rid * NS + sub) < 0).any())
        seg_len = np.bincount(rid * NS + sub, minlength=n * NS)
    if unsorted:
        raise AssertionError("class rows must have their edges sorted by (xcd_subclass(column), column)")
    seg_e0 = np.repeat(rowptr[rows], NS) + (np.cumsum(seg_len) - seg_len - np.repeat(start, NS))
    nchunk = -(-seg_len // chunk)
    tot = int(nchunk.sum())
    if items_per_block is None:
        items_per_block = items_per_block_for(tot)
    seg_of = np.repeat(np.arange(n * NS), nchunk)
    within = np.arange(tot, dtype=np.int64) - np.repeat(np.cumsum(nchunk) - nchunk, nchunk)
    e0 = seg_e0[seg_of] + within * chunk
    ln = np.minimum(chunk, seg_len[seg_of] - within * chunk)
    slot_ptr = np.zeros(n + 1, dtype=np.int64)
    np.cumsum(nchunk.reshape(n, NS).sum(1), out=slot_ptr[1:])
    item_cls = (seg_of % NS) % XCD_CLASSES
    heavy = sizes > phase_threshold if (phases > 1 and phase_threshold > 0) else np.zeros(n, dtype=bool)
    mega = ((sizes > mega_segment_edges * XCD_CLASSES * np.where(heavy, max(1, phases), 1)) & (sizes >= mega_min_edges)) \
        if mega_segment_edges > 0 else np.zeros(n, dtype=bool)
    item_group = np.where(heavy[seg_of // NS], (seg_of % NS) // XCD_CLASSES, max(1, phases))
    ids = (rows if row_ids is None else row_ids).astype(np.int32)
    item_row = ids[seg_of // NS]
    pieces = []
    for g in range(max(1, phases) + 1):
        in_group = item_group == g
        if not in_group.any():
            continue
        per_class = [np.nonzero(in_group & (item_cls == c))[0] for c in range(XCD_CLASSES)]
        if mega.any():
            ordered = []
            for pc in per_class:
                is_mega = mega[seg_of[pc] // NS]
                first = pc[is_mega]
                ordered.append(np.concatenate([first[np.argsort(colidx[e0[first]], kind="stable")], pc[~is_mega]]))
            per_class = ordered
        nblk = max(-(-len(pc) // items_per_block) for pc in per_class)
        flat = XCD_CLASSES * nblk * items_per_block
        g_e0 = np.zeros(flat, dtype=np.int64)
        g_len = np.zeros(flat, dtype=np.int32)
        g_slot = np.full(flat, -1, dtype=np.int32)
        g_row = np.zeros(flat, dtype=np.int32)
        for c, pc in enumerate(per_class):
            t = np.arange(len(pc))
            where = (t // items_per_block) * (XCD_CLASSES * items_per_block) + c * items_per_block + t % items_per_block
            g_e0[where], g_len[where], g_slot[where], g_row[where] = e0[pc], ln[pc], pc, item_row[pc]
        pieces.append((g_e0, g_len, g_slot, g_row))
    if not pieces:
        flat = XCD_CLASSES * items_per_block
        pieces.append((np.zeros(flat, dtype=np.int64), np.zeros(flat, dtype=np.int32),
                       np.full(flat, -1, dtype=np.int32), np.zeros(flat, dtype=np.int32)))
    out_e0, out_len, out_slot, out_row = (np.concatenate([p[i] for p in pieces]) for i in range(4))
    return {"e0": out_e0, "len": out_len, "slot": out_slot, "row": out_row, "slot_ptr": slot_ptr,
            "items_per_block": int(items_per_block)}


def items_per_block_for(n_items: int) -> int:
    return int(min(CLASS_ITEMS_PER_BLOCK, max(4, 4 * -(-n_items // (4 * 4096)))))
```

include/clane_hip.h:

```cpp
#ifndef CLANE_HIP_H_
#define CLANE_HIP_H_

#include <stdint.h>

#ifdef __cplusplus
extern "C" {
#endif

#define CLANE_ABI_VERSION 5

#define CLANE_OK 0
#define CLANE_ERR_INVALID_ARGUMENT (-1)
#define CLANE_ERR_LAUNCH (-2)

#define CLANE_SCORE_REFERENCE 0
#define CLANE_SCORE_PER_EDGE 1
#define CLANE_SCORE_RAW_DOT 2

#define CLANE_SCORE_FUSE_SOFTMAX 1
#define CLANE_SCORE_ROW_PARTS(n) (((n) & 0xff) << 8)

#define CLANE_SPMM_SINKS_UNTOUCHED 1
#define CLANE_SPMM_TABLE_BEYOND_CACHE 2

// ... 56 lines not shown
int clane_spmm_update_f32(const int64_t *rowptr, const int32_t *colidx, const float *P, int64_t nrows, int64_t row0,
                          const float *Z_old, int64_t ldz, const float *X, int64_t ldx, float gamma, float *Z_new,
                          int64_t ldo, int32_t d, int64_t long_threshold, int32_t flags, const clane_mirror_t *mirror,
                          double *delta_partials, void *stream);
int clane_spmm_update_f64(const int64_t *rowptr, const int32_t *colidx, const double *P, int64_t nrows, int64_t row0,
                          const double *Z_old, int64_t ldz, const double *X, int64_t ldx, double gamma, double *Z_new,
                          int64_t ldo, int32_t d, int64_t long_threshold, int32_t flags, const clane_mirror_t *mirror,
                          double *delta_partials, void *stream);
int clane_spmm_update_bf16(const int64_t *rowptr, const int32_t *colidx, const float *P, int64_t nrows, int64_t row0,
                           const uint16_t *Z_old, int64_t ldz, const uint16_t *X, int64_t ldx, float gamma,
                           uint16_t *Z_new, int64_t ldo, int32_t d, int64_t long_threshold, int32_t flags,
                           const clane_mirror_t *mirror, double *delta_partials, void *stream);
int clane_spmm_update_long_f32(const int64_t *rowptr, const int32_t *colidx, const float *P, const int32_t *long_rows,
                               int64_t n_long, int32_t waves_per_row, int64_t row0, const float *Z_old, int64_t ldz, const float *X,
                               int64_t ldx, float gamma, float *Z_new, int64_t ldo, int32_t d,
                               const clane_mirror_t *mirror, double *delta_partials, void *stream);
int clane_spmm_update_long_f64(const int64_t *rowptr, const int32_t *colidx, const double *P,
                               const int32_t *long_rows, int64_t n_long, int32_t waves_per_row, int64_t row0, const double *Z_old,
                               int64_t ldz, const double *X, int64_t ldx, double gamma, double *Z_new, int64_t ldo,
                               int32_t d, const clane_mirror_t *mirror, double *delta_partials, void *stream);
int clane_spmm_update_long_bf16(const int64_t *rowptr, const int32_t *colidx, const float *P,
                                const int32_t *long_rows, int64_t n_long, int32_t waves_per_row, int64_t row0, const uint16_t *Z_old,
                                int64_t ldz, const uint16_t *X, int64_t ldx, float gamma, uint16_t *Z_new,
                                int64_t ldo, int32_t d, const clane_mirror_t *mirror, double *delta_partials,
                                void *stream);

int64_t clane_spmm_split_slab_len(int64_t n_segments, int32_t d);
int clane_spmm_update_split_f32(const int64_t *rowptr, const int32_t *colidx, const float *P, const int32_t *split_rows,
                                const int64_t *seg_ptr, const int32_t *seg_row, int64_t n_split, int64_t n_segments,
                                int64_t edges_per_segment, int64_t row0, const float *Z_old, int64_t ldz,
                                const float *X, int64_t ldx, float gamma, float *Z_new, int64_t ldo, int32_t d,
                                float *slab, const clane_mirror_t *mirror, double *delta_partials, void *stream);
int clane_spmm_update_split_f64(const int64_t *rowptr, const int32_t *colidx, const double *P,
                                const int32_t *split_rows, const int64_t *seg_ptr, const int32_t *seg_row,
                                int64_t n_split, int64_t n_segments, int64_t edges_per_segment, int64_t row0,
                                const double *Z_old, int64_t ldz, const double *X, int64_t ldx, double gamma,
                                double *Z_new, int64_t ldo, int32_t d, double *slab, const clane_mirror_t *mirror,
                                double *delta_partials, void *stream);
int clane_spmm_update_split_bf16(const int64_t *rowptr, const int32_t *colidx, const float *P,
                                 const int32_t *split_rows, const int64_t *seg_ptr, const int32_t *seg_row,
                                 int64_t n_split, int64_t n_segments, int64_t edges_per_segment, int64_t row0,
                                 const uint16_t *Z_old, int64_t ldz, const uint16_t *X, int64_t ldx, float gamma,
                                 uint16_t *Z_new, int64_t ldo, int32_t d, float *slab, const clane_mirror_t *mirror,
                                 double *delta_partials, void *stream);

int clane_edge_score_class_f32(const int64_t *rowptr, const int32_t *colidx, const int64_t *item_e0,
                               const int32_t *item_len, const int32_t *item_slot, const int32_t *item_row,
                               int64_t n_blocks, int32_t items_per_block, const int32_t *class_rows,
                               const int64_t *slot_ptr, int64_t n_rows, int64_t row0, const float *Z, int64_t ldz,
                               int32_t d, int32_t mode, const double *sums2, const float *sq, float *scores,
                               int32_t flags, float *stats, void *stream);
int clane_edge_score_class_f64(const int64_t *rowptr, const int32_t *colidx, const int64_t *item_e0,
                               const int32_t *item_len, const int32_t *item_slot, const int32_t *item_row,
                               int64_t n_blocks, int32_t items_per_block, const int32_t *class_rows,
                               const int64_t *slot_ptr, int64_t n_rows, int64_t row0, const double *Z, int64_t ldz,
                               int32_t d, int32_t mode, const double *sums2, const double *sq, double *scores,
                               int32_t flags, double *stats, void *stream);
int clane_edge_score_class_bf16(const int64_t *rowptr, const int32_t *colidx, const int64_t *item_e0,
                                const int32_t *item_len, const int32_t *item_slot, const int32_t *item_row,
                                int64_t n_blocks, int32_t items_per_block, const int32_t *class_rows,
                                const int64_t *slot_ptr, int64_t n_rows, int64_t row0, const uint16_t *Z, int64_t ldz,
                                int32_t d, int32_t mode, const double *sums2, const float *sq, float *scores,
                                int32_t flags, float *stats, void *stream);

int64_t clane_spmm_class_slab_len(int64_t n_slots, int32_t d);
int clane_spmm_update_class_f32(const int32_t *colidx, const float *P, const int64_t *item_e0, const int32_t *item_len,
                                const int32_t *item_slot, int64_t n_blocks, int32_t items_per_block,
                                const int32_t *class_rows, const int64_t *slot_ptr, int64_t n_rows, int64_t row0,
                                const float *Z_old, int64_t ldz, const float *X, int64_t ldx, float gamma, float *Z_new,
                                int64_t ldo, int32_t d, int32_t flags, float *slab, const clane_mirror_t *mirror,
                                double *delta_partials, void *stream);
int clane_spmm_update_class_f64(const int32_t *colidx, const double *P, const int64_t *item_e0, const int32_t *item_len,
                                const int32_t *item_slot, int64_t n_blocks, int32_t items_per_block,
                                const int32_t *class_rows, const int64_t *slot_ptr, int64_t n_rows, int64_t row0,
                                const double *Z_old, int64_t ldz, const double *X, int64_t ldx, double gamma,
                                double *Z_new, int64_t ldo, int32_t d, int32_t flags, double *slab, const clane_mirror_t *mirror,
                                double *delta_partials, void *stream);
int clane_spmm_update_class_bf16(const int32_t *colidx, const float *P, const int64_t *item_e0, const int32_t *item_len,
                                 const int32_t *item_slot, int64_t n_blocks, int32_t items_per_block,
                                 const int32_t *class_rows, const int64_t *slot_ptr, int64_t n_rows, int64_t row0,
                                 const uint16_t *Z_old, int64_t ldz, const uint16_t *X, int64_t ldx, float gamma,
                                 uint16_t *Z_new, int64_t ldo, int32_t d, int32_t flags, float *slab, const clane_mirror_t *mirror,
                                 double *delta_partials, void *stream);

int clane_reduce_partials(const double *partials, int64_t n, double *ws, double *out, void *stream);

int clane_l1_distance_f32(const float *A, int64_t lda, const float *B, int64_t ldb, int64_t nrows, int32_t d,
                          float *sq_a, double *ws, double *out, void *stream);
int clane_l1_distance_f64(const double *A, int64_t lda, const double *B, int64_t ldb, int64_t nrows, int32_t d,
                          double *sq_a, double *ws, double *out, void *stream);
int clane_l1_distance_bf16(const uint16_t *A, int64_t lda, const uint16_t *B, int64_t ldb, int64_t nrows, int32_t d,
                           float *sq_a, double *ws, double *out, void *stream);

int clane_gather_rows_f32(const float *src, int64_t lds, const int32_t *idx, int64_t n, int32_t d, float *dst,
                          int64_t ldd, void *stream);
int clane_gather_rows_f64(const double *src, int64_t lds, const int32_t *idx, int64_t n, int32_t d, double *dst,
                          int64_t ldd, void *stream);
int clane_gather_rows_bf16(const uint16_t *src, int64_t lds, const int32_t *idx, int64_t n, int32_t d, uint16_t *dst,
                           int64_t ldd, void *stream);

int clane_pair_cosine_f32(const float *A, int64_t lda, const float *B, int64_t ldb, int64_t nrows, int32_t d,
                          float *out, double *ws, void *stream);
int clane_pair_cosine_f64(const double *A, int64_t lda, const double *B, int64_t ldb, int64_t nrows, int32_t d,
                          double *out, double *ws, void *stream);

int clane_project_rows_f32(const float *Z, int64_t rows, int32_t d, int64_t ldz, const float *W, float *Y, int64_t ldy,
                           void *stream);
int clane_project_rows_f64(const double *Z, int64_t rows, int32_t d, int64_t ldz, const double *W, double *Y,
                           int64_t ldy, void *stream);
int clane_project_rows_bf16(const uint16_t *Z, int64_t rows, int32_t d, int64_t ldz, const float *W, float *Y,
                            int64_t ldy, void *stream);

int clane_edge_score_pair_f32(const int64_t *rowptr, const int32_t *colidx, int64_t nrows, int64_t row0, const float *S,
                              int64_t lds, const float *N, int64_t ldn, int32_t d, float *scores, int32_t flags,
                              int64_t long_threshold, const int32_t *long_rows, int64_t n_long, void *stream);
int clane_edge_score_pair_f64(const int64_t *rowptr, const int32_t *colidx, int64_t nrows, int64_t row0,
                              const double *S, int64_t lds, const double *N, int64_t ldn, int32_t d, double *scores,
                              int32_t flags, int64_t long_threshold, const int32_t *long_rows, int64_t n_long,
                              void *stream);
int clane_edge_score_class_pair_f32(const int64_t *rowptr, const int32_t *colidx, const int64_t *item_e0,
                                    const int32_t *item_len, const int32_t *item_slot, const int32_t *item_row,
                                    int64_t n_blocks, int32_t items_per_block, const int32_t *class_rows,
                                    const int64_t *slot_ptr, int64_t n_rows, int64_t row0, const float *S, int64_t lds,
                                    const float *N, int64_t ldn, int32_t d, float *scores, int32_t flags, float *stats,
                                    void *stream);
int clane_edge_score_class_pair_f64(const int64_t *rowptr, const int32_t *colidx, const int64_t *item_e0,
                                    const int32_t *item_len, const int32_t *item_slot, const int32_t *item_row,
                                    int64_t n_blocks, int32_t items_per_block, const int32_t *class_rows,
                                    const int64_t *slot_ptr, int64_t n_rows, int64_t row0, const double *S,
                                    int64_t lds, const double *N, int64_t ldn, int32_t d, double *scores,
                                    int32_t flags, double *stats, void *stream);

int clane_pair_project_f32(const float *Z, int64_t table_rows, int32_t d, int64_t ldz, const int32_t *src,
                           const int32_t *dst, int64_t B, const float *W, float *A, float *Bm, void *stream);
int clane_pair_project_f64(const double *Z, int64_t table_rows, int32_t d, int64_t ldz, const int32_t *src,
                           const int32_t *dst, int64_t B, const double *W, double *A, double *Bm, void *stream);
int clane_pair_project_bf16(const uint16_t *Z, int64_t table_rows, int32_t d, int64_t ldz, const int32_t *src,
                            const int32_t *dst, int64_t B, const float *W, float *A, float *Bm, void *stream);
int clane_pair_loss_f32(const float *A, const float *Bm, int64_t B, int32_t d, const uint8_t *linked, const float *u,
                        float *g, uint8_t *mask, double *ws, double *stats, void *stream);
int clane_pair_loss_f64(const double *A, const double *Bm, int64_t B, int32_t d, const uint8_t *linked, const double *u,
                        double *g, uint8_t *mask, double *ws, double *stats, void *stream);
int64_t clane_pair_grad_ws_len(int64_t B, int32_t d);
int clane_pair_grad_f32(const float *Z, int64_t table_rows, int32_t d, int64_t ldz, const int32_t *src,
                        const int32_t *dst, int64_t B, const float *A, const float *Bm, const float *g,
                        const double *stats, float *ws, float *dW, void *stream);
int clane_pair_grad_f64(const double *Z, int64_t table_rows, int32_t d, int64_t ldz, const int32_t *src,
                        const int32_t *dst, int64_t B, const double *A, const double *Bm, const double *g,
                        const double *stats, double *ws, double *dW, void *stream);
int clane_pair_grad_bf16(const uint16_t *Z, int64_t table_rows, int32_t d, int64_t ldz, const int32_t *src,
                         const int32_t *dst, int64_t B, const float *A, const float *Bm, const float *g,
                         const double *stats, float *ws, float *dW, void *stream);
int clane_adam_step_f32(float *W, float *m, float *v, const float *dW, int64_t n, double lr, const double *stats,
                        double *state, void *stream);
int clane_adam_step_f64(double *W, double *m, double *v, const double *dW, int64_t n, double lr, const double *stats,
                        double *state, void *stream);
int clane_pair_labels(const int64_t *rowptr, const int32_t *colidx, int64_t nrows, const int32_t *src,
                      const int32_t *dst, int64_t B, uint8_t *linked, void *stream);

#define CLANE_RANK_MAX_K 32
int clane_rank_scores_f32(const float *S, int64_t lds, const float *N, int64_t ldn, int64_t table_rows, int32_t d,
                          const int32_t *q_rows, int64_t Q, int32_t mode, const double *sums2, const float *sq,
                          const int32_t *label, const int64_t *excl_rowptr, const int32_t *excl_colidx,
                          int32_t exclude_self, int32_t k, int32_t n_slabs, float *cand_score, int32_t *cand_id,
                          void *stream);
int clane_rank_scores_f64(const double *S, int64_t lds, const double *N, int64_t ldn, int64_t table_rows, int32_t d,
// ... 143 lines not shown
```

Measured before the change: 274.9 sweeps/s.

## Add owned-row SpMM kernel accumulating virtual-row partial sums in LDS

Adds an owned-plan SpMM update path. Each block (one of a fixed number of groups) owns a set of rows, split into virtual rows, and accumulates their partial sums in a large dynamic LDS buffer. It walks the XCD column-class segments step by step, and waves claim segments through an LDS atomic counter. This is meant to replace the slab and global-partials scheme of the class kernel, removing its extra global writes and reduction and improving cache locality per column class. In exchange it needs a host-side greedy planner and close to the full LDS per CU, which limits occupancy to one block per CU.

```diff
diff --git a/clane_amd/_hip.py b/clane_amd/_hip.py
--- a/clane_amd/_hip.py
+++ b/clane_amd/_hip.py
@@ -59,6 +59,8 @@
         C.c_int, [_p, _p, _p, _p, _p, _p, _i64, _i32, _p, _p, _i64, _i64, _p, _i64, _i32, _i32, _p, _p, _p, _i32, _p, _p])
     SIGNATURES[f"clane_gather_rows_{_s}"] = (C.c_int, [_p, _i64, _p, _i64, _i32, _p, _i64, _p])
     SIGNATURES[f"clane_l1_distance_{_s}"] = (C.c_int, [_p, _i64, _p, _i64, _i64, _i32, _p, _p, _p, _p])
+SIGNATURES["clane_spmm_update_owned_f32"] = (
+    C.c_int, [_p, _p, _p, _i32, _i64, _p, _i64, _p, _i64, C.c_float, _p, _i64, _i32, _i32, _p, _p])
 for _s in ("f32", "f64"):
     SIGNATURES[f"clane_degree_weighted_sums_{_s}"] = (C.c_int, [_p, _p, _p, _i64, _p, _p, _p])
     SIGNATURES[f"clane_edge_score_finalize_{_s}"] = (C.c_int, [_p, _p, _i64, _i64, _i32, _p, _p, _p, _p])
@@ -239,6 +241,60 @@
             pass
 
 
+class _OwnedPlanStruct(C.Structure):
+    _fields_ = [(name, _p) for name in ("grp_bat_ptr", "bat_vrow_ptr", "bat_row_ptr", "bat_seg_ptr", "seg_e0", "seg_len",
+                                        "seg_vrow", "row_id", "row_part", "row_vptr")] + \
+               [(name, _i32) for name in ("n_groups", "n_steps", "chunk", "max_batch_vrows")]
+
+
+OWNED_PLAN_ARRAYS = {"grp_bat_ptr": torch.int32, "bat_vrow_ptr": torch.int32, "bat_row_ptr": torch.int32,
+                     "bat_seg_ptr": torch.int32, "seg_e0": torch.int64, "seg_len": torch.int32, "seg_vrow": torch.int32,
+                     "row_id": torch.int32, "row_part": torch.int32, "row_vptr": torch.int32}
+OWNED_MAX_STEPS = 64
+OWNED_LDS_LIMIT = 159 * 1024
+
+
+class OwnedPlan:
+
+    def __init__(self, plan: dict, chunk: int, device):
+        self.n_groups, self.n_steps = int(plan["n_groups"]), int(plan["n_steps"])
+        self.chunk, self.max_batch_vrows = int(chunk), int(plan["max_batch_vrows"])
+        self.n_rows = int(plan["row_id"].shape[0])
+        self.arrays = {}
+        for name, dtype in OWNED_PLAN_ARRAYS.items():
+            t = torch.as_tensor(plan[name])
+            if t.dtype != dtype or t.dim() != 1:
+                raise ValueError(f"OwnedPlan: {name} must be a 1-D {dtype} array")
+            self.arrays[name] = t.contiguous().to(device)
+        a = {k: v.cpu() for k, v in self.arrays.items()}
+        B = a["bat_vrow_ptr"].numel() - 1
+        ok = (a["grp_bat_ptr"].numel() == self.n_groups + 1 and int(a["grp_bat_ptr"][0]) == 0
+              and int(a["grp_bat_ptr"][-1]) == B and bool((a["grp_bat_ptr"].diff() >= 0).all())
+              and a["bat_row_ptr"].numel() == B + 1 and a["bat_seg_ptr"].numel() == B * self.n_steps + 1
+              and int(a["bat_vrow_ptr"][0]) == 0 and int(a["bat_row_ptr"][0]) == 0 and int(a["bat_seg_ptr"][0]) == 0
+              and bool((a["bat_vrow_ptr"].diff() >= 0).all()) and bool((a["bat_row_ptr"].diff() >= 0).all())
+              and bool((a["bat_seg_ptr"].diff() >= 0).all()) and int(a["bat_row_ptr"][-1]) == self.n_rows
+              and a["row_vptr"].numel() == self.n_rows + 1 and a["row_part"].numel() == self.n_rows
+              and int(a["row_vptr"][0]) == 0 and bool((a["row_vptr"].diff() >= 1).all())
+              and int(a["row_vptr"][-1]) == int(a["bat_vrow_ptr"][-1])
+              and bool((a["row_vptr"][a["bat_row_ptr"].long()] == a["bat_vrow_ptr"]).all())
+              and int(a["bat_vrow_ptr"].diff().max() if B else 0) <= self.max_batch_vrows
+              and a["seg_e0"].numel() == a["seg_len"].numel() == a["seg_vrow"].numel() == int(a["bat_seg_ptr"][-1])
+              and 1 <= self.n_steps <= OWNED_MAX_STEPS and self.chunk >= 64 and self.chunk % 64 == 0)
+        if ok and a["seg_len"].numel():
+            per_batch = a["bat_seg_ptr"][self.n_steps::self.n_steps] - a["bat_seg_ptr"][:-1:self.n_steps]
+            seg_bat = torch.repeat_interleave(torch.arange(B), per_batch.long())
+            ok = bool((a["seg_len"] > 0).all()) and bool((a["seg_e0"] >= 0).all()) and bool((a["seg_vrow"] >= 0).all()) \
+                and bool((a["seg_vrow"] < a["bat_vrow_ptr"].diff()[seg_bat]).all())
+        if not ok:
+            raise ValueError("OwnedPlan: the arrays do not describe a plan (see include/clane_hip.h)")
+        self.max_edge = int((a["seg_e0"] + a["seg_len"]).max()) if a["seg_len"].numel() else 0
+        self.max_row = int(a["row_id"].max()) if self.n_rows else -1
+        self.max_part = int(a["row_part"].max()) if self.n_rows else -1
+        self.c = _OwnedPlanStruct(*[self.arrays[name].data_ptr() for name in OWNED_PLAN_ARRAYS], self.n_groups,
+                                  self.n_steps, self.chunk, self.max_batch_vrows)
+
+
 def _mirror_arg(mirror: Optional["Mirror"], dtype: torch.dtype):
     if mirror is None:
         return None
@@ -430,6 +486,16 @@
 
     def project_affine(self, Z, d: int, rows, mu, W, Y):
         raise NotImplementedError(f"{type(self).__name__} has no project_affine")
+
+    def has_spmm_owned(self, dtype, d: int) -> bool:
+        return False
+
+    def make_owned_plan(self, plan: dict, chunk: int, device):
+        raise NotImplementedError(f"{type(self).__name__} has no make_owned_plan")
+
+    def spmm_update_owned(self, colidx, P, plan, block_threads: int, row0: int, Z_old, X, gamma: float, Z_new, d: int,
+                          partials, beyond_cache: bool = False, loads: int = 0):
+        raise NotImplementedError(f"{type(self).__name__} has no spmm_update_owned")
 
     def bind(self, method: str, *args, **kwargs):
         fn = getattr(self, method)
@@ -638,6 +704,31 @@
                      class_rows.numel(), row0, zo, ldz, xp, ldx, gamma, zn, ldo, d,
                      SPMM_TABLE_BEYOND_CACHE if beyond_cache else 0,
                      _vec(slab, acc_dtype(Z_old.dtype), "slab"), _mirror_arg(mirror, Z_new.dtype),
+                     _vec(partials, torch.float64, "partials"), self._stream(Z_old))
+
+    def has_spmm_owned(self, dtype, d: int) -> bool:
+        return dtype == torch.float32 and 64 < d <= 256
+
+    def make_owned_plan(self, plan: dict, chunk: int, device) -> OwnedPlan:
+        return OwnedPlan(plan, chunk, device)
+
+    def spmm_update_owned(self, colidx, P, plan: OwnedPlan, block_threads: int, row0: int, Z_old, X, gamma: float,
+                          Z_new, d: int, partials, beyond_cache: bool = False, loads: int = 0):
+        zo, ldz = _mat(Z_old, "Z_old")
+        xp, ldx = _mat(X, "X")
+        zn, ldo = _mat(Z_new, "Z_new")
+        if not (Z_old.dtype == X.dtype == Z_new.dtype == torch.float32):
+            raise TypeError("spmm_update_owned: float32 tables only")
+        lanes = 32 if d <= 128 else 64
+        if plan.max_batch_vrows * lanes * 16 > OWNED_LDS_LIMIT:
+            raise ValueError(f"spmm_update_owned: {plan.max_batch_vrows} virtual rows per batch do not fit the LDS")
+        if (plan.max_edge > min(colidx.numel(), P.numel()) or plan.max_row >= min(X.shape[0], Z_new.shape[0])
+                or row0 + plan.max_row >= Z_old.shape[0] or plan.max_part >= partials.numel()):
+            raise ValueError("spmm_update_owned: the plan reaches outside colidx / P, the tables or the partials")
+        self._invoke(self.lib.clane_spmm_update_owned_f32, "clane_spmm_update_owned",
+                     _vec(colidx, torch.int32, "colidx"), _vec(P, torch.float32, "P"), C.cast(C.pointer(plan.c), _p),
+                     int(block_threads), row0, zo, ldz, xp, ldx, gamma, zn, ldo, d,
+                     (SPMM_TABLE_BEYOND_CACHE if beyond_cache else 0) | ((int(loads) & 0xff) << 8),
                      _vec(partials, torch.float64, "partials"), self._stream(Z_old))
 
     def reduce_partials(self, partials, n: int, ws, out):
diff --git a/clane_amd/csrc/clane_abi.hip b/clane_amd/csrc/clane_abi.hip
--- a/clane_amd/csrc/clane_abi.hip
+++ b/clane_amd/csrc/clane_abi.hip
@@ -499,6 +499,77 @@
     return check_launch("spmm_update_class");
 }
 
+constexpr int64_t kOwnedLdsReserve = 1024;
+constexpr int64_t kLdsPerCU = 160 * 1024;
+constexpr int64_t kLdsDefaultLimit = 64 * 1024;
+
+template <typename T, typename PT>
+int spmm_update_owned(const int32_t *colidx, const PT *P, const clane_owned_plan_t *plan, int32_t block_threads,
+                      int64_t row0, const T *Z_old, int64_t ldz, const T *X, int64_t ldx,
+                      typename Elem<T>::acc_t gamma, T *Z_new, int64_t ldo, int32_t d, int32_t flags,
+                      double *delta_partials, void *stream) {
+    using A = typename Elem<T>::acc_t;
+    REQUIRE(plan, "spmm_update_owned: null plan");
+    REQUIRE(plan->n_groups >= 0 && row0 >= 0 && d > 0, "spmm_update_owned: bad shape");
+    REQUIRE(plan->n_steps >= 1 && plan->n_steps <= kOwnedMaxSteps, "spmm_update_owned: n_steps must be in [1, %d]",
+            kOwnedMaxSteps);
+    REQUIRE(plan->chunk >= kWave && plan->chunk % kWave == 0, "spmm_update_owned: chunk must be a positive multiple of 64");
+    REQUIRE(block_threads >= kWave && block_threads <= kOwnedMaxBlock && block_threads % kWave == 0,
+            "spmm_update_owned: block_threads must be a multiple of 64 in [64, %d]", kOwnedMaxBlock);
+    REQUIRE(ldz >= d && ldx >= d && ldo >= d, "spmm_update_owned: leading dimension < d");
+    REQUIRE(plan->max_batch_vrows >= 0, "spmm_update_owned: negative max_batch_vrows");
+    if (plan->n_groups == 0) return CLANE_OK;
+    REQUIRE(colidx && P && plan->grp_bat_ptr && plan->bat_vrow_ptr && plan->bat_row_ptr && plan->bat_seg_ptr &&
+                plan->seg_e0 && plan->seg_len && plan->seg_vrow && plan->row_id && plan->row_part && plan->row_vptr &&
+                Z_old && X && Z_new && delta_partials,
+            "spmm_update_owned: null pointer");
+    REQUIRE((const void *)Z_new != (const void *)Z_old, "spmm_update_owned: Z_new must not alias Z_old");
+    const Layout L = pick_layout<T>(d, {Z_old, X, Z_new}, {ldz, ldx, ldo});
+    REQUIRE(L.vec && (L.lpr == 32 || L.lpr == 64) && d <= L.lpr * Elem<T>::kVec,
+            "spmm_update_owned: no instance for d=%d with these operands (16-byte packs, 17..64 packs per row)", d);
+    const int64_t lds = int64_t(plan->max_batch_vrows) * L.lpr * Elem<T>::kVec * int64_t(sizeof(A));
+    REQUIRE(lds + kOwnedLdsReserve <= kLdsPerCU, "spmm_update_owned: %lld virtual rows per batch need %lld bytes of LDS",
+            (long long)plan->max_batch_vrows, (long long)lds);
+    const OwnedPlan op{plan->grp_bat_ptr, plan->bat_vrow_ptr, plan->bat_row_ptr, plan->bat_seg_ptr, plan->seg_e0,
+                       plan->seg_len, plan->seg_vrow, plan->row_id, plan->row_part, plan->row_vptr, plan->n_steps,
+                       plan->chunk};
+    const bool beyond = (flags & CLANE_SPMM_TABLE_BEYOND_CACHE) != 0;
+    int rc = CLANE_OK;
+    auto launch = [&]<int VEC, int LPR, int U>() {
+        auto *kernel = spmm_owned_kernel<T, PT, VEC, LPR, U>;
+        if (lds > kLdsDefaultLimit) {
+            static int64_t granted = 0;
+            if (lds > granted) {
+                const hipError_t e = hipFuncSetAttribute(reinterpret_cast<const void *>(kernel),
+                                                         hipFuncAttributeMaxDynamicSharedMemorySize, int(lds));
+                if (e != hipSuccess) {
+                    rc = fail(CLANE_ERR_LAUNCH, "spmm_update_owned: %lld bytes of LDS: %s", (long long)lds,
+                              hipGetErrorString(e));
+                    return;
+                }
+                granted = lds;
+            }
+        }
+        kernel<<<unsigned(plan->n_groups), unsigned(block_threads), size_t(lds), (hipStream_t)stream>>>(
+            colidx, P, op, row0, Z_old, ldz, X, ldx, gamma, Z_new, ldo, d, beyond, delta_partials);
+    };
+    constexpr int KV = Elem<T>::kVec;
+    const int asked = (flags >> 8) & 0xff;
+    REQUIRE(asked == 0 || asked == 8 || asked == 12 || (L.lpr == 32 && asked == 6),
+            "spmm_update_owned: no instance with %d row loads in flight", asked);
+    const int loads = asked ? asked : (L.lpr == 32 && beyond) ? CLANE_CLASS_U32 : CLANE_LONG_U;
+    if (L.lpr == 32) {
+        if (loads == 6) launch.template operator()<KV, 32, 6>();
+        else if (loads == 12) launch.template operator()<KV, 32, 12>();
+        else launch.template operator()<KV, 32, 8>();
+    } else {
+        if (loads == 12) launch.template operator()<KV, 64, 12>();
+        else launch.template operator()<KV, 64, 8>();
+    }
+    if (rc != CLANE_OK) return rc;
+    return check_launch("spmm_update_owned");
+}
+
 template <typename T>
 int l1_distance(const T *A, int64_t lda, const T *B, int64_t ldb, int64_t nrows, int32_t d,
                 typename Elem<T>::acc_t *sq_a, double *ws, double *out, void *stream) {
@@ -1212,6 +1283,13 @@
 CLANE_CLASS_WRAPPER(f64, double, double, double, double)
 CLANE_CLASS_WRAPPER(bf16, uint16_t, bf16_t, float, float)
 #undef CLANE_CLASS_WRAPPER
+int clane_spmm_update_owned_f32(const int32_t *colidx, const float *P, const clane_owned_plan_t *plan,
+                                int32_t block_threads, int64_t row0, const float *Z_old, int64_t ldz, const float *X,
+                                int64_t ldx, float gamma, float *Z_new, int64_t ldo, int32_t d, int32_t flags,
+                                double *delta_partials, void *stream) {
+    return spmm_update_owned<float, float>(colidx, P, plan, block_threads, row0, Z_old, ldz, X, ldx, gamma, Z_new, ldo,
+                                           d, flags, delta_partials, stream);
+}
 int64_t clane_spmm_class_slab_len(int64_t n_slots, int32_t d) { return n_slots * (ceil_div(d, 8) * 8); }
 int64_t clane_spmm_split_slab_len(int64_t n_segments, int32_t d) { return n_segments * (ceil_div(d, 8) * 8); }
 
diff --git a/clane_amd/csrc/spmm_update.h b/clane_amd/csrc/spmm_update.h
--- a/clane_amd/csrc/spmm_update.h
+++ b/clane_amd/csrc/spmm_update.h
@@ -752,4 +752,134 @@
     }
 }
 
-}
+constexpr int kOwnedMaxSteps = 64;
+constexpr int kOwnedMaxBlock = 1024;
+
+struct OwnedPlan {
+    const int32_t *grp_bat_ptr;
+    const int32_t *bat_vrow_ptr;
+    const int32_t *bat_row_ptr;
+    const int32_t *bat_seg_ptr;
+    const int64_t *seg_e0;
+    const int32_t *seg_len;
+    const int32_t *seg_vrow;
+    const int32_t *row_id;
+    const int32_t *row_part;
+    const int32_t *row_vptr;
+    int n_steps;
+    int chunk;
+};
+
+template <typename T, typename PT, int VEC, int LPR, int U>
+__global__ __launch_bounds__(kOwnedMaxBlock) void spmm_owned_kernel(
+    const int32_t *__restrict__ colidx, const PT *__restrict__ P, OwnedPlan plan, int64_t row0,
+    const T *__restrict__ Zold, int64_t ldz, const T *__restrict__ X, int64_t ldx, typename Elem<T>::acc_t gamma,
+    T *__restrict__ Znew, int64_t ldo, int d, bool nt_store, double *__restrict__ partials) {
+    using A = typename Elem<T>::acc_t;
+    constexpr int W = LPR * VEC;
+    constexpr int kRows = kWave / LPR;
+    extern __shared__ __align__(16) unsigned char s_owned_raw[];
+    A *s_sum = reinterpret_cast<A *>(s_owned_raw);
+    __shared__ int s_cnt[kOwnedMaxSteps];
+
+    const int lane = lane_id();
+    const int wave = __builtin_amdgcn_readfirstlane(threadIdx.x / kWave);
+    const int nwaves = int(blockDim.x) / kWave;
+    const int sub = lane / LPR, sl = lane % LPR;
+    const int c0 = sl * VEC;
+    const bool col_ok = c0 < d;
+    const T *zcol = Zold + (col_ok ? c0 : 0);
+    const int n_steps = plan.n_steps;
+    const int64_t chunk = plan.chunk;
+    const int b0 = plan.grp_bat_ptr[blockIdx.x], b1 = plan.grp_bat_ptr[blockIdx.x + 1];
+
+    for (int b = b0; b < b1; ++b) {
+        const int v0 = plan.bat_vrow_ptr[b];
+        const int nv = plan.bat_vrow_ptr[b + 1] - v0;
+        for (int i = threadIdx.x; i < nv * W; i += int(blockDim.x)) s_sum[i] = A(0);
+        if (int(threadIdx.x) < n_steps) s_cnt[threadIdx.x] = 0;
+        __syncthreads();
+        for (int s = 0; s < n_steps; ++s) {
+            const int sa = plan.bat_seg_ptr[b * n_steps + s];
+            const int n = plan.bat_seg_ptr[b * n_steps + s + 1] - sa;
+            auto claim = [&]() -> int {
+                int v = 0;
+                if (lane == 0) v = atomicAdd(&s_cnt[s], 1);
+                return __builtin_amdgcn_readfirstlane(v);
+            };
+            int cur = claim();
+            int64_t e0 = 0, e1 = 0;
+            int vr = 0;
+            EdgeChunk<A> ch{0, A(0)};
+            if (cur < n) {
+                e0 = plan.seg_e0[sa + cur];
+                e1 = e0 + plan.seg_len[sa + cur];
+                vr = plan.seg_vrow[sa + cur];
+                ch = load_chunk<A, PT>(colidx, P, e0, e0 + chunk < e1 ? e0 + chunk : e1);
+            }
+            while (cur < n) {
+                const int nxt = claim();
+                int64_t n0 = 0, n1 = 0;
+                int vn = 0;
+                EdgeChunk<A> chn{0, A(0)};
+                if (nxt < n) {
+                    n0 = plan.seg_e0[sa + nxt];
+                    n1 = n0 + plan.seg_len[sa + nxt];
+                    vn = plan.seg_vrow[sa + nxt];
+                    chn = load_chunk<A, PT>(colidx, P, n0, n0 + chunk < n1 ? n0 + chunk : n1);
+                }
+                A *sum = s_sum + vr * W + c0;
+                for (int64_t p = e0; p < e1; p += chunk) {
+                    const int64_t pe = p + chunk < e1 ? p + chunk : e1;
+                    A acc[VEC];
+#pragma unroll
+                    for (int k = 0; k < VEC; ++k) acc[k] = A(0);
+                    gather_accumulate<T, PT, VEC, LPR, U>(colidx, P, p, pe, zcol, ldz, col_ok, acc, ch, p == e0);
+                    fold_subwaves<LPR>(acc);
+                    if (col_ok && sub == 0) {
+                        Pack<A, VEC> t = load_pack<A, VEC>(sum);
+#pragma unroll
+                        for (int k = 0; k < VEC; ++k) t.v[k] += acc[k];
+                        store_pack<A, VEC>(sum, t);
+                    }
+                }
+                cur = nxt;
+                e0 = n0;
+                e1 = n1;
+                vr = vn;
+                ch = chn;
+            }
+            __syncthreads();
+        }
+        const int r0 = plan.bat_row_ptr[b];
+        const int nr = plan.bat_row_ptr[b + 1] - r0;
+        for (int j0 = wave * kRows; j0 < nr; j0 += nwaves * kRows) {
+            const int j = j0 + sub;
+            const bool live = j < nr;
+            const bool ok = live && col_ok;
+            A rsum = A(0);
+            if (ok) {
+                const int64_t r = plan.row_id[r0 + j];
+                const Pack<T, VEC> x = load_pack_stream<T, VEC>(X + r * ldx + c0);
+                const Pack<T, VEC> zo = load_pack_stream<T, VEC>(Zold + (row0 + r) * ldz + c0);
+                const int va = plan.row_vptr[r0 + j] - v0, vb = plan.row_vptr[r0 + j + 1] - v0;
+                A acc[VEC];
+                const Pack<A, VEC> first = load_pack<A, VEC>(s_sum + va * W + c0);
+#pragma unroll
+                for (int k = 0; k < VEC; ++k) acc[k] = first.v[k];
+                for (int v = va + 1; v < vb; ++v) {
+                    const Pack<A, VEC> t = load_pack<A, VEC>(s_sum + v * W + c0);
+#pragma unroll
+                    for (int k = 0; k < VEC; ++k) acc[k] += t.v[k];
+                }
+                Pack<T, VEC> out{};
+                rsum = finish_pack<T, VEC>(x, zo, acc, gamma, true, Znew + r * ldo + c0, out, nt_store);
+            }
+            rsum = group_sum<LPR>(rsum);
+            if (live && sl == 0) partials[plan.row_part[r0 + j]] = double(rsum);
+        }
+        __syncthreads();
+    }
+}
+
+}
diff --git a/clane_amd/diagnostics.py b/clane_amd/diagnostics.py
--- a/clane_amd/diagnostics.py
+++ b/clane_amd/diagnostics.py
@@ -43,7 +43,8 @@
         narrow = self.d > 0 and lanes_per_row(self.d_plan if len(self.tiles) > 1 else self.d, self.dtype) < 64
         return {"main": "spmm_update_subrow_kernel" if narrow else "spmm_update_kernel",
                 "mid": "spmm_long_kernel<4 waves>", "hub": "spmm_long_kernel<16 waves>",
-                "split": "spmm_class_chunk_kernel+combine" if self.class_threshold > 0
+                "split": ("spmm_owned_kernel+spmm_class_chunk_kernel+combine" if getattr(self, "class_owned", False)
+                          else "spmm_class_chunk_kernel+combine") if self.class_threshold > 0
                 else "spmm_split_segment_kernel+combine"}
 
     def estimated_sweep_seconds(self) -> float:
@@ -68,6 +69,11 @@
                 "fewer_loads_in_flight": bool(self.beyond_cache and self.d > 0 and (str(self.dtype), lanes_per_row(
                     self.d_plan if len(self.tiles) > 1 else self.d, self.dtype)) in (("torch.float32", 32), ("torch.bfloat16", 16))),
                 "hot_rows_first": self.hot_rows_first, "exchange": self.exchange,
+                **({"class_owned": {"max_edges": self.owned_max_edges, "row_edges": self.owned_row_edges,
+                                    "groups": self.owned_groups, "block_threads": self.owned_block_threads,
+                                    "batch_vrows": self.owned_batch_vrows, "chunk": self.owned_chunk,
+                                    "loads": self.owned_loads}}
+                   if getattr(self, "class_owned", False) else {}),
                 }
 
     def exchange_bytes_per_sweep(self) -> int:
diff --git a/clane_amd/engine.py b/clane_amd/engine.py
--- a/clane_amd/engine.py
+++ b/clane_amd/engine.py
@@ -7,7 +7,7 @@
 import numpy as np
 import torch
 
-from . import _hip, xcd
+from . import _hip, owned, xcd
 from .comm import TorchComm
 from .diagnostics import DiagnosticsMixin
 from .halo import build_halo_layout
@@ -34,7 +34,11 @@
                  overlap_chunks: bool = True, fused_pack: bool = True, class_threshold: Optional[int] = None,
                  class_chunk: int = CLASS_CHUNK, class_k1: bool = True, class_phases: Optional[int] = None,
                  phase_threshold: int = PHASE_THRESHOLD, delta_stream: bool = False, table_skew=None,
-                 table_alloc: str = "torch", column_tiles: Optional[int] = None):
+                 table_alloc: str = "torch", column_tiles: Optional[int] = None, class_owned: Optional[bool] = None,
+                 owned_max_edges: int = xcd.OWNED_MAX_EDGES, owned_row_edges: int = xcd.OWNED_ROW_EDGES,
+                 owned_groups: int = xcd.OWNED_GROUPS, owned_lds_bytes: int = xcd.OWNED_LDS_BYTES,
+                 owned_block_threads: int = xcd.OWNED_BLOCK_THREADS, owned_chunk: Optional[int] = None,
+                 owned_loads: int = xcd.OWNED_LOADS):
         if X.dim() != 2 or X.shape[0] != csr.num_vertices:
             raise ValueError(f"X must be [V, d] with V={csr.num_vertices}, got {tuple(X.shape)}")
         if cosine_mode not in ("reference", "per_edge"):
@@ -53,6 +57,9 @@
         self._column_tiles_asked = column_tiles
         X = self._choose_division(csr, X, process_group, comm, exchange)
         self._choose_class_pass(csr, class_threshold, class_chunk, class_k1, class_phases, phase_threshold)
+        self._choose_owned(class_owned, owned_max_edges, owned_row_edges, owned_groups, owned_lds_bytes,
+                           owned_block_threads, owned_chunk)
+        self.owned_loads = int(owned_loads)
         self._build_layout(csr, chunks, shuffle, seed, hot_rows_first)
         self._choose_row_bins(long_threshold, hub_threshold)
         deg = self._upload_structure()
@@ -147,6 +154,31 @@
             raise ValueError("class_chunk must be a multiple of 64 in [64, 4096]")
         self.mega_segment_edges = int(L2_BYTES_ALL_XCDS // 8 // max(row_bytes, 1)) if self.d_plan > 0 else 0
 
+    def _choose_owned(self, class_owned, max_edges, row_edges, groups, lds_bytes, block_threads, chunk) -> None:
+        can = owned.possible(self)
+        want = (xcd.OWNED_DEFAULT and self.beyond_cache and self.class_affinity) if class_owned is None else bool(class_owned)
+        self.class_owned, self.owned_possible = bool(want and can), bool(can)
+        self._lds_bytes = int(lds_bytes)
+        self.owned_max_edges, self.owned_row_edges = int(max_edges), int(row_edges)
+        self.owned_groups, self.owned_block_threads = int(groups), int(block_threads)
+        self.owned_chunk = int(chunk) if chunk is not None else self.class_chunk
+        if self.class_owned:
+            self._check_owned_settings()
+
+    def _check_owned_settings(self) -> None:
+        widths = [c1 - c0 for c0, c1 in self.tiles]
+        if self.owned_groups < 1 or self.owned_row_edges < 64 or not (
+                64 <= self.owned_block_threads <= 1024 and self.owned_block_threads % 64 == 0):
+            raise ValueError("owned_groups must be >= 1, owned_row_edges >= 64, owned_block_threads a multiple of 64 "
+                             "in [64, 1024]")
+        if not (64 <= self.owned_chunk <= 4096 and self.owned_chunk % 64 == 0):
+            raise ValueError("owned_chunk must be a multiple of 64 in [64, 4096]")
+        sum_bytes = 16 * lanes_per_row(max(widths), self.dtype)
+        self.owned_batch_vrows = self._lds_bytes // sum_bytes
+        if self.owned_batch_vrows < 1 or self.owned_batch_vrows * sum_bytes > _hip.OWNED_LDS_LIMIT:
+            raise ValueError(f"owned_lds_bytes must hold one sum of {sum_bytes} bytes and stay within "
+                             f"{_hip.OWNED_LDS_LIMIT}")
+
     def _build_layout(self, csr: HostCSR, chunks, shuffle, seed: int, hot_rows_first: bool) -> None:
         if chunks is None:
             chunks = 1 if self.row_world == 1 else 4
@@ -211,6 +243,8 @@
         self.split_rows: List[Optional[tuple]] = []
         self.class_rows: List[Optional[tuple]] = []
         self.class_slots: List[int] = []
+        self.owned_rows: List[Optional[tuple]] = []
+        self._owned_inputs = {}
         self.k1_long_rows: List[Optional[torch.Tensor]] = []
         self.split_edges = SPLIT_EDGES if split_hubs else 0
         hub_edges = int(deg[deg > SPLIT_EDGES].sum()) // max(1, len(self.blocks))
@@ -234,8 +268,13 @@
                 phased = dict(phase_threshold=self.phase_threshold, phases=self.class_phases,
                               mega_segment_edges=self.mega_segment_edges,
                               mega_min_edges=self.part.padded_vertices // 4)
+                segments = xcd.row_segments(self.local.rowptr, self.local.colidx, rows_abs, self.colidx,
+                                            self.phase_threshold, self.class_phases)
                 items = class_items(self.local.rowptr, self.local.colidx, rows_abs, self.class_chunk, None,
-                                    row_ids=rows_c, colidx_dev=self.colidx, **phased)
+                                    row_ids=rows_c, colidx_dev=self.colidx, segments=segments, **phased)
+                self.owned_rows.append(owned.plan_block(self, rows_c, rows_abs, segments, phased) if self.class_owned else None)
+                if self.owned_possible:
+                    self._owned_inputs[len(self.owned_rows) - 1] = (rows_c, rows_abs, segments, phased)
                 ipb = items["items_per_block"]
                 self.class_rows.append((to_dev(rows_c), torch.from_numpy(items["slot_ptr"]).to(dev),
                                         torch.from_numpy(items["e0"]).to(dev), torch.from_numpy(items["len"]).to(dev),
@@ -246,6 +285,7 @@
             else:
                 self.class_rows.append(None)
                 self.class_slots.append(0)
+                self.owned_rows.append(None)
             k1_long = (db > self.k1_threshold) & ~(is_class if self.class_k1 else np.zeros_like(is_class)) \
                 if self.k1_threshold > 0 else np.zeros_like(is_class)
             self.k1_long_rows.append(to_dev(np.nonzero(k1_long)[0]))
@@ -268,6 +308,25 @@
             slab_len = max(slab_len, self.k.spmm_class_slab_len(max_slots, max(self.d_plan, 1)), 2 * max_slots)
         self.slabs = [torch.zeros(slab_len, dtype=self.acc_dtype, device=dev)
                       for _ in range(2 if len(self.blocks) > 1 else 1)]
+
+    def set_owned(self, on: bool, **settings) -> None:
+        if on and not self.owned_possible:
+            raise ValueError("this engine has no owned pass: one GPU, fp32, rows or tiles of 65..256 elements")
+        if self.device.type == "cuda":
+            torch.cuda.synchronize(self.device)
+        for name, value in settings.items():
+            if name == "lds_bytes":
+                self._lds_bytes = int(value)
+            elif name in ("max_edges", "row_edges", "groups", "block_threads", "chunk", "loads"):
+                setattr(self, "owned_" + name, int(value))
+            else:
+                raise TypeError(f"set_owned: unknown setting {name!r}")
+        self.class_owned = bool(on)
+        if on:
+            self._check_owned_settings()
+        self.owned_rows = [owned.plan_block(self, *self._owned_inputs[i]) if on and i in self._owned_inputs else None
+                           for i in range(len(self.blocks))]
+        self._plans = {}
 
     def _setup_exchange(self, deg: np.ndarray, fused_pack: bool) -> None:
         dev = self.device
@@ -583,7 +642,18 @@
                 if mir is not None and T > 1:
                     raise AssertionError("column tiles and mirrored launches do not combine")
                 for t in range(T):
-                    if self.class_rows[i] is not None:
+                    if self.owned_rows[i] is not None:
+                        plan, rest, _ = self.owned_rows[i]
+                        steps.append(("call", owned.bind_launch(self, plan, b.row0, cut(Zold, t), cut(Xb, t), gamma,
+                                                                cut(Zn, t), width(t), part(po_class, t))))
+                        if rest is not None:
+                            rows_r, slot_ptr, it_e0, it_len, it_slot, ipb = rest
+                            steps.append(("call", self._bind("spmm_update_class", self.colidx, self.P, it_e0, it_len,
+                                                             it_slot, ipb, rows_r, slot_ptr, b.row0, cut(Zold, t),
+                                                             cut(Xb, t), gamma, cut(Zn, t), width(t),
+                                                             self.slabs[i % len(self.slabs)], part(po_class, t),
+                                                             mirror=mir, beyond_cache=self.beyond_cache)))
+                    elif self.class_rows[i] is not None:
                         rows_c, slot_ptr, it_e0, it_len, it_slot, _, ipb = self.class_rows[i]
                         steps.append(("call", self._bind("spmm_update_class", self.colidx, self.P, it_e0, it_len, it_slot,
                                                          ipb, rows_c, slot_ptr, b.row0, cut(Zold, t), cut(Xb, t), gamma,
diff --git a/clane_amd/owned.py b/clane_amd/owned.py
--- /dev/null
+++ b/clane_amd/owned.py
@@ -0,0 +1,44 @@
+from __future__ import annotations
+
+from typing import Optional
+
+import numpy as np
+import torch
+
+from . import xcd
+
+
+def possible(eng) -> bool:
+    widths = [c1 - c0 for c0, c1 in eng.tiles]
+    return bool(eng.world == 1 and not eng._forced and eng.class_threshold > 0 and eng.d > 0
+                and all(eng.k.has_spmm_owned(eng.dtype, w) for w in widths))
+
+
+def plan_block(eng, rows_c: np.ndarray, rows_abs: np.ndarray, segments, phased: dict) -> Optional[tuple]:
+    dev = eng.device
+    sizes, seg_len, seg_e0 = segments
+    NS = seg_len.size // max(1, sizes.size)
+    own = sizes <= eng.owned_max_edges
+    if not own.any():
+        return None
+    n_rest = int((~own).sum())
+    pick = lambda a, m: a.reshape(sizes.size, NS)[m].reshape(-1)
+    plan = xcd.owned_plan(sizes[own], pick(seg_len, own), pick(seg_e0, own), rows_c[own],
+                          n_rest + np.arange(int(own.sum())), row_edges=eng.owned_row_edges,
+                          groups=eng.owned_groups, batch_vrows=eng.owned_batch_vrows)
+    eng.owned_balance = plan["group_step_edges"]
+    rest = None
+    if n_rest:
+        keep = ~own
+        items = xcd.class_items(eng.local.rowptr, eng.local.colidx, rows_abs[keep], eng.class_chunk, None,
+                                row_ids=rows_c[keep], segments=(sizes[keep], pick(seg_len, keep), pick(seg_e0, keep)),
+                                **phased)
+        rest = (torch.from_numpy(rows_c[keep].astype(np.int32)).to(dev), torch.from_numpy(items["slot_ptr"]).to(dev),
+                torch.from_numpy(items["e0"]).to(dev), torch.from_numpy(items["len"]).to(dev),
+                torch.from_numpy(items["slot"]).to(dev), items["items_per_block"])
+    return eng.k.make_owned_plan(plan, eng.owned_chunk, dev), rest, n_rest
+
+
+def bind_launch(eng, plan, row0: int, Zold, Xb, gamma: float, Zn, width: int, partials):
+    return eng._bind("spmm_update_owned", eng.colidx, eng.P, plan, eng.owned_block_threads, row0, Zold, Xb, gamma, Zn,
+                     width, partials, beyond_cache=eng.beyond_cache, loads=eng.owned_loads)
diff --git a/clane_amd/xcd.py b/clane_amd/xcd.py
--- a/clane_amd/xcd.py
+++ b/clane_amd/xcd.py
@@ -42,37 +42,12 @@
 
 def class_items(rowptr: np.ndarray, colidx: np.ndarray, rows: np.ndarray, chunk: int, items_per_block: Optional[int],
                 row_ids: Optional[np.ndarray] = None, colidx_dev: Optional[torch.Tensor] = None,
-                phase_threshold: int = 0, phases: int = 1, mega_segment_edges: int = 0, mega_min_edges: int = 0) -> dict:
+                phase_threshold: int = 0, phases: int = 1, mega_segment_edges: int = 0, mega_min_edges: int = 0,
+                segments=None) -> dict:
     n = rows.size
     NS = XCD_CLASSES * max(1, phases)
-    sizes = (rowptr[rows + 1] - rowptr[rows]).astype(np.int64)
-    start = np.concatenate([[0], np.cumsum(sizes)[:-1]])
-    if colidx_dev is not None and colidx_dev.is_cuda:
-        dev = colidx_dev.device
-        seg_len = np.empty(n * NS, dtype=np.int64)
-        unsorted = False
-        bounds = np.concatenate([[0], np.cumsum(sizes)])
-        for a, b in row_pieces(bounds, CLASS_ITEMS_PIECE_EDGES):
-            if bounds[b] == bounds[a]:
-                seg_len[a * NS:b * NS] = 0
-                continue
-            sizes_t = torch.from_numpy(sizes[a:b]).to(dev)
-            rid = torch.repeat_interleave(torch.arange(b - a, device=dev), sizes_t)
-            idx = (torch.from_numpy(rowptr[rows[a:b]] - (start[a:b] - bounds[a])).to(dev)[rid]
-                   + torch.arange(int(bounds[b] - bounds[a]), device=dev))
-            sub = xcd_subclass(colidx_dev[idx].long(), sizes_t[rid], 0, phase_threshold, phases)
-            key = rid * NS + sub
-            unsorted = unsorted or (bool((key[1:] < key[:-1]).any()) if key.numel() > 1 else False)
-            seg_len[a * NS:b * NS] = torch.bincount(key, minlength=(b - a) * NS).cpu().numpy()
-    else:
-        idx = np.repeat(rowptr[rows] - start, sizes) + np.arange(int(sizes.sum()), dtype=np.int64)
-        rid = np.repeat(np.arange(n, dtype=np.int64), sizes)
-        sub = xcd_subclass(colidx[idx].astype(np.int64), sizes[rid], 0, phase_threshold, phases)
-        unsorted = idx.size > 1 and bool((np.diff(rid * NS + sub) < 0).any())
-        seg_len = np.bincount(rid * NS + sub, minlength=n * NS)
-    if unsorted:
-        raise AssertionError("class rows must have their edges sorted by (xcd_subclass(column), column)")
-    seg_e0 = np.repeat(rowptr[rows], NS) + (np.cumsum(seg_len) - seg_len - np.repeat(start, NS))
+    sizes, seg_len, seg_e0 = segments if segments is not None else \
+        row_segments(rowptr, colidx, rows, colidx_dev, phase_threshold, phases)
     nchunk = -(-seg_len // chunk)
     tot = int(nchunk.sum())
     if items_per_block is None:
@@ -123,5 +98,125 @@
             "items_per_block": int(items_per_block)}
 
 
+def row_segments(rowptr: np.ndarray, colidx: np.ndarray, rows: np.ndarray, colidx_dev: Optional[torch.Tensor] = None,
+                 phase_threshold: int = 0, phases: int = 1):
+    n = rows.size
+    NS = XCD_CLASSES * max(1, phases)
+    sizes = (rowptr[rows + 1] - rowptr[rows]).astype(np.int64)
+    start = np.concatenate([[0], np.cumsum(sizes)[:-1]])
+    if colidx_dev is not None and colidx_dev.is_cuda:
+        dev = colidx_dev.device
+        seg_len = np.empty(n * NS, dtype=np.int64)
+        unsorted = False
+        bounds = np.concatenate([[0], np.cumsum(sizes)])
+        for a, b in row_pieces(bounds, CLASS_ITEMS_PIECE_EDGES):
+            if bounds[b] == bounds[a]:
+                seg_len[a * NS:b * NS] = 0
+                continue
+            sizes_t = torch.from_numpy(sizes[a:b]).to(dev)
+            rid = torch.repeat_interleave(torch.arange(b - a, device=dev), sizes_t)
+            idx = (torch.from_numpy(rowptr[rows[a:b]] - (start[a:b] - bounds[a])).to(dev)[rid]
+                   + torch.arange(int(bounds[b] - bounds[a]), device=dev))
+            sub = xcd_subclass(colidx_dev[idx].long(), sizes_t[rid], 0, phase_threshold, phases)
+            key = rid * NS + sub
+            unsorted = unsorted or (bool((key[1:] < key[:-1]).any()) if key.numel() > 1 else False)
+            seg_len[a * NS:b * NS] = torch.bincount(key, minlength=(b - a) * NS).cpu().numpy()
+    else:
+        idx = np.repeat(rowptr[rows] - start, sizes) + np.arange(int(sizes.sum()), dtype=np.int64)
+        rid = np.repeat(np.arange(n, dtype=np.int64), sizes)
+        sub = xcd_subclass(colidx[idx].astype(np.int64), sizes[rid], 0, phase_threshold, phases)
+        unsorted = idx.size > 1 and bool((np.diff(rid * NS + sub) < 0).any())
+        seg_len = np.bincount(rid * NS + sub, minlength=n * NS)
+    if unsorted:
+        raise AssertionError("class rows must have their edges sorted by (xcd_subclass(column), column)")
+    seg_e0 = np.repeat(rowptr[rows], NS) + (np.cumsum(seg_len) - seg_len - np.repeat(start, NS))
+    return sizes, seg_len.astype(np.int64), seg_e0
+
+
 def items_per_block_for(n_items: int) -> int:
     return int(min(CLASS_ITEMS_PER_BLOCK, max(4, 4 * -(-n_items // (4 * 4096)))))
+
+
+OWNED_MAX_EDGES = 512
+OWNED_ROW_EDGES = 1024
+OWNED_GROUPS = 256
+OWNED_BLOCK_THREADS = 1024
+OWNED_LDS_BYTES = 152 * 1024
+OWNED_LOADS = 12
+OWNED_DEFAULT = True
+
+
+def owned_plan(sizes: np.ndarray, seg_len: np.ndarray, seg_e0: np.ndarray, row_ids: np.ndarray, row_parts: np.ndarray,
+               *, row_edges: int, groups: int, batch_vrows: int) -> Optional[dict]:
+    n = int(sizes.size)
+    if n == 0:
+        return None
+    if groups < 1 or row_edges < 64:
+        raise ValueError("owned_plan: groups must be >= 1 and row_edges >= 64")
+    NS = seg_len.size // n
+    seg_len = seg_len.reshape(n, NS).astype(np.int64)
+    seg_e0 = seg_e0.reshape(n, NS).astype(np.int64)
+    keys = np.nonzero(seg_len.sum(0) > 0)[0]
+    if keys.size == 0:
+        keys = np.zeros(1, dtype=np.int64)
+    S = int(keys.size)
+    seg_len, seg_e0 = seg_len[:, keys], seg_e0[:, keys]
+    nv = np.maximum(1, -(-sizes // row_edges)).astype(np.int64)
+    while True:
+        over = (-(-seg_len // nv[:, None])).sum(1) > row_edges
+        if not over.any():
+            break
+        nv[over] += 1
+    if int(nv.max()) > batch_vrows:
+        raise ValueError(f"owned_plan: a row of {int(nv.max())} virtual rows does not fit a batch of {batch_vrows}")
+    row_cum = np.cumsum(seg_len, 1).astype(np.float64)
+    share = np.maximum(row_cum.sum(0) / groups, 1.0)
+    row_cum /= share
+    cum = np.zeros((groups, S))
+    group_of = np.empty(n, dtype=np.int64)
+    dealt = np.argsort(-sizes, kind="stable")
+    for i in dealt.tolist():
+        g = int((cum + row_cum[i]).max(1).argmin())
+        group_of[i] = g
+        cum[g] += row_cum[i]
+    order = dealt[np.argsort(group_of[dealt], kind="stable")]
+    g_sorted, nv_sorted = group_of[order], nv[order]
+    bat_of_row = np.empty(n, dtype=np.int64)
+    b, used, g_prev = -1, 0, -1
+    for j, (g, k) in enumerate(zip(g_sorted.tolist(), nv_sorted.tolist())):
+        if g != g_prev or used + k > batch_vrows:
+            b, used, g_prev = b + 1, 0, g
+        used += k
+        bat_of_row[j] = b
+    B = b + 1
+    bat_row_ptr = np.zeros(B + 1, dtype=np.int64)
+    np.cumsum(np.bincount(bat_of_row, minlength=B), out=bat_row_ptr[1:])
+    row_vptr = np.zeros(n + 1, dtype=np.int64)
+    np.cumsum(nv_sorted, out=row_vptr[1:])
+    bat_vrow_ptr = row_vptr[bat_row_ptr]
+    bat_group = g_sorted[bat_row_ptr[:-1]]
+    grp_bat_ptr = np.zeros(groups + 1, dtype=np.int64)
+    np.cumsum(np.bincount(bat_group, minlength=groups), out=grp_bat_ptr[1:])
+    nvirt = int(row_vptr[-1])
+    v_row = np.repeat(np.arange(n), nv_sorted)
+    v_j = np.arange(nvirt) - row_vptr[v_row]
+    L, E0, NV = seg_len[order][v_row], seg_e0[order][v_row], nv_sorted[v_row][:, None]
+    lo = (v_j[:, None] * L) // NV
+    hi = ((v_j[:, None] + 1) * L) // NV
+    v_len, v_e0 = hi - lo, E0 + lo
+    v_idx, s_idx = np.nonzero(v_len > 0)
+    v_bat = bat_of_row[v_row]
+    key = v_bat[v_idx] * S + s_idx
+    by = np.lexsort((v_idx, key))
+    v_idx, s_idx, key = v_idx[by], s_idx[by], key[by]
+    bat_seg_ptr = np.zeros(B * S + 1, dtype=np.int64)
+    np.cumsum(np.bincount(key, minlength=B * S), out=bat_seg_ptr[1:])
+    group_step = np.zeros((groups, S), dtype=np.int64)
+    np.add.at(group_step, (g_sorted[v_row][v_idx], s_idx), v_len[v_idx, s_idx])
+    i32 = lambda a: np.ascontiguousarray(a, dtype=np.int32)
+    return {"grp_bat_ptr": i32(grp_bat_ptr), "bat_vrow_ptr": i32(bat_vrow_ptr), "bat_row_ptr": i32(bat_row_ptr),
+            "bat_seg_ptr": i32(bat_seg_ptr), "seg_e0": np.ascontiguousarray(v_e0[v_idx, s_idx], dtype=np.int64),
+            "seg_len": i32(v_len[v_idx, s_idx]), "seg_vrow": i32(v_idx - bat_vrow_ptr[v_bat[v_idx]]),
+            "row_id": i32(row_ids[order]), "row_part": i32(row_parts[order]), "row_vptr": i32(row_vptr),
+            "n_groups": int(groups), "n_steps": S, "max_batch_vrows": int(np.diff(bat_vrow_ptr).max()),
+            "steps": keys.astype(np.int64), "group_step_edges": group_step}
diff --git a/include/clane_hip.h b/include/clane_hip.h
--- a/include/clane_hip.h
+++ b/include/clane_hip.h
@@ -162,6 +162,28 @@
                                  const uint16_t *Z_old, int64_t ldz, const uint16_t *X, int64_t ldx, float gamma,
                                  uint16_t *Z_new, int64_t ldo, int32_t d, int32_t flags, float *slab, const clane_mirror_t *mirror,
                                  double *delta_partials, void *stream);
+
+#define CLANE_OWNED_LOADS(n) (((n) & 0xff) << 8)
+typedef struct {
+    const int32_t *grp_bat_ptr;
+    const int32_t *bat_vrow_ptr;
+    const int32_t *bat_row_ptr;
+    const int32_t *bat_seg_ptr;
+    const int64_t *seg_e0;
+    const int32_t *seg_len;
+    const int32_t *seg_vrow;
+    const int32_t *row_id;
+    const int32_t *row_part;
+    const int32_t *row_vptr;
+    int32_t n_groups;
+    int32_t n_steps;
+    int32_t chunk;
+    int32_t max_batch_vrows;
+} clane_owned_plan_t;
+int clane_spmm_update_owned_f32(const int32_t *colidx, const float *P, const clane_owned_plan_t *plan,
+                                int32_t block_threads, int64_t row0, const float *Z_old, int64_t ldz, const float *X,
+                                int64_t ldx, float gamma, float *Z_new, int64_t ldo, int32_t d, int32_t flags,
+                                double *delta_partials, void *stream);
 
 int clane_reduce_partials(const double *partials, int64_t n, double *ws, double *out, void *stream);
 
```

Measured after the change: 283.7 sweeps/s (median of 6 runs). +3.2%, better.
